# msyriac/orphics

Measured on AMD Instinct MI355X. Metric: QE kappa reconstructions/sec on 8192^2 maps, higher is better.
Workload: dtype f64

## Files before the change

### include/orphics_amd.h

```cpp
#ifndef ORPHICS_AMD_H
#define ORPHICS_AMD_H

#include <stddef.h>
#include <stdint.h>

#ifdef __cplusplus
extern "C" {
#endif

#define OA_F32 0
#define OA_F64 1

typedef struct oa_plan oa_plan;

const char* oa_last_error(void);
#define OA_ABI_VERSION 409
int oa_version(void);
int oa_device_count(void);

int oa_plan_create(int ny, int nx, int dtype, oa_plan** out);
int oa_plan_destroy(oa_plan* p);
long oa_plan_kpitch(const oa_plan* p);
long oa_plan_scratch_bytes(const oa_plan* p);
int oa_plan_set_laxes(oa_plan* p, const double* host_ly, const double* host_lx);

int oa_fft_r2c(oa_plan* p, const void* real_in, void* hc_out, double scale, int width, int rband, void* stream);
int oa_fft_c2r(oa_plan* p, const void* hc_in, void* real_out, double scale, int width, void* stream);
int oa_fft_c2r_windowed(oa_plan* p, const void* hc_in, void* real_out, double scale, const void* window_real, void* stream);
int oa_fft_c2c(oa_plan* p, const void* full_in, void* full_out, int inverse, double scale, void* stream);
int oa_fft_pass(oa_plan* p, int pass_id, const void* in, void* out, int width, void* stream);

int oa_fft_cols(oa_plan* p, const void* hc_in, void* hc_out, int inverse, double scale, int width, void* stream);
int oa_qe_rows(oa_plan* p, const void* gx, const void* gy, const void* h, void* px, void* py, double scale,
               int accumulate, int win, int wout, int mrow, void* stream);

int oa_qe_legs_cols(oa_plan* p, const void* kX, const void* kY, const void* FG, const void* FH, void* gx, void* gy, void* h,
                    int width, int rband, void* stream);
int oa_qe_map_legs_cols(oa_plan* p, const void* real_map, const void* FG, const void* FH, void* gx, void* gy, void* h,
                        int width, int rband, void* stream);
int oa_qe_cols_div(oa_plan* p, const void* px_rows, const void* py_rows, const void* Fnorm, void* out, int accumulate,
                   int width, int rband, void* stream);

int oa_plan_set_filters(oa_plan* p, const void* FG, const void* FH, const void* Fnorm, int leg_cols, int kappa_cols,
                        int leg_rows, int kappa_rows, int mrow);
int oa_plan_set_col_grid(oa_plan* p, int mcol);
int oa_plan_col_grid(const oa_plan* p);
int oa_plan_band_grid(const oa_plan* p, int* my, int* mx);
int oa_qe_band_bind(oa_plan* p, int nfilters, const void* const* host_filters, int nnorms, const void* const* host_Fnorm, int leg_cols,
                    int kappa_cols, int leg_rows, int kappa_rows, int mrow, int mcol, int max_leg_planes);
int oa_qe_band_grid(const oa_plan* p, int* my, int* mx);
int oa_plan_rsplit(const oa_plan* p);
int oa_plan_div_fused(const oa_plan* p);
enum { OA_OPT_MC_BATCH = 1, OA_OPT_MV_BATCH = 2, OA_OPT_MV_ROWBATCH = 3, OA_OPT_MV_CHAIN = 4, OA_OPT_DIV_BIN = 5, OA_OPT_WIN_FUSED = 6 };
int oa_plan_set_option(oa_plan* p, int option, int value);
int oa_plan_set_bins(oa_plan* p, const int32_t* ids_hc, int nids, double norm, void* stream);
void* oa_plan_kappa(oa_plan* p);
const int64_t* oa_plan_bin_counts(oa_plan* p);
int oa_qe_tt(oa_plan* p, const void* real_map, const void* kX, const void* kY, void* out_kappa_hc, int zero_outside,
             void* stream);
int oa_qe_pol(oa_plan* p, int npieces, const double* host_signs, const void* const* host_FG, const void* const* host_FH,
              const int* host_swap, const void* kX, const void* kY, const void* Fnorm, void* out, int accumulate,
              int leg_cols, int kappa_cols, int leg_rows, int kappa_rows, int mrow, int zero_outside, void* stream);
int oa_qe_mv(oa_plan* p, int nest, const int* host_npieces, const double* host_signs, const void* const* host_FG,
             const void* const* host_FH, const int* host_swap, const void* const* host_kX, const void* const* host_kY,
             const void* const* host_Fnorm, void* out, int accumulate, int leg_cols, int kappa_cols, int leg_rows, int kappa_rows,
             int mrow, int zero_outside, void* stream);
int oa_qe_mv_maps(oa_plan* p, int nmaps, const void* const* host_maps, const void* rot_c, const void* rot_s, int nest,
                  const int* host_npieces, const double* host_signs, const void* const* host_FG, const void* const* host_FH,
                  const int* host_swap, const int* host_xsrc, const int* host_ysrc, const void* const* host_Fnorm, void* out,
                  int accumulate, int leg_cols, int kappa_cols, int leg_rows, int kappa_rows, int mrow, int zero_outside, void* stream);
int oa_filter_map(oa_plan* p, const void* real_in, const void* filt_hcreal, void* real_out, void* stream);
int oa_qe_tt_moments(oa_plan* p, const void* real_map, int64_t* n, double* S, double* C, void* stream);
int oa_qe_tt_moments2(oa_plan* p, const void* real_map0, const void* real_map1, int64_t* n, double* S, double* C, void* stream);
int oa_qe_tt_splits(oa_plan* p, int nsplits, const void* const* host_kmaps, void* const* host_out, int zero_outside, void* stream);
int oa_qe_tt_split_power(oa_plan* p, int nsplits, const void* const* host_kmaps, void* out_hcreal, double norm, int zero_outside,
                         void* stream);
int oa_split_cross_power(int dtype, int nsplits, const void* const* host_kappa, void* out_hcreal, double norm, int ny, long kpitch,
                         int active_cols, int active_rows, void* stream);
int oa_mc_run(oa_plan* p, uint64_t base_seed, long sim_lo, long sim_hi, const void* covsqrt_hc, int64_t* n, double* S,
              double* C, double* meanfield_acc, void* stream);
int oa_mc_run_windowed(oa_plan* p, uint64_t base_seed, long sim_lo, long sim_hi, const void* covsqrt_hc, const void* window_real,
                       int64_t* n, double* S, double* C, double* meanfield_acc, void* stream);
int oa_mc_mv_band_bind(oa_plan* p, const void* mv_weights, long mv_wstride, int nest, const int32_t* ids_hc, int nids, int nspec_max);
int oa_mc_run_mv(oa_plan* p, uint64_t base_seed, long sim_lo, long sim_hi, const void* const* host_covsqrt, int nest, const int* host_npieces,
                 const double* host_signs, const void* const* host_FG, const void* const* host_FH, const int* host_swap, const int* host_xsrc,
                 const int* host_ysrc, const void* const* host_Fnorm, const void* mv_weights, long mv_wstride, int nspec, const int* host_a,
                 const int* host_b, const int32_t* ids_hc, int nids, const int64_t* counts, double norm, int leg_cols, int kappa_cols,
                 int leg_rows, int kappa_rows, int mrow, int64_t* n, double* S, double* C, void* stream);
int oa_mc_run_mv_windowed(oa_plan* p, uint64_t base_seed, long sim_lo, long sim_hi, const void* const* host_covsqrt, int nest,
                          const int* host_npieces, const double* host_signs, const void* const* host_FG, const void* const* host_FH,
                          const int* host_swap, const int* host_xsrc, const int* host_ysrc, const void* const* host_Fnorm, const void* mv_weights,
                          long mv_wstride, int nspec, const int* host_a, const int* host_b, const int32_t* ids_hc, int nids, const int64_t* counts,
                          double norm, int leg_cols, int kappa_cols, int leg_rows, int kappa_rows, int mrow, const void* window_real,
                          const void* rot_c, const void* rot_s, int64_t* n, double* S, double* C, double* const* host_meanfield, void* stream);
int oa_qe_tt_stage(oa_plan* p, int stage, const void* real_map, void* stream);

int oa_malloc(void** out, size_t bytes);
int oa_free(void* dptr);
int oa_memcpy(void* dst, const void* src, size_t bytes, int kind, void* stream);
int oa_memset(void* dptr, int value, size_t bytes, void* stream);
int oa_stream_synchronize(void* stream);

int oa_comm_unique_id(void* id128);
int oa_comm_init(int nranks, int rank, const void* id128, void** comm_out);
int oa_comm_destroy(void* comm);
int oa_allreduce(void* comm, void* device_buf, long count, int dtype_code, void* stream);

int oa_hc_to_full(oa_plan* p, const void* hc_in, void* full_out, void* stream);
int oa_full_to_hc(oa_plan* p, const void* full_in, void* hc_out, void* stream);
int oa_hcreal_to_full(oa_plan* p, const void* hcreal_in, void* fullreal_out, void* stream);
int oa_fullreal_to_hc(oa_plan* p, const void* fullreal_in, void* hcreal_out, void* stream);

int oa_f2power(int dtype, const void* k1, const void* k2, void* out_real, double norm, long n, void* stream);
int oa_cmul_real(int dtype, const void* k_in, const void* filt_real, void* k_out, long n, void* stream);
int oa_cmul(int dtype, const void* k_in, const void* filt_complex, void* k_out, long n, void* stream);
int oa_mul_real(int dtype, const void* a, const void* b, void* out, long n, void* stream);
int oa_axpby_real(int dtype, const void* a, const void* b, void* out, double alpha, double beta, long n, void* stream);
int oa_rot2(int dtype, const void* c, const void* s, const void* i1, const void* i2, void* o1, void* o2, long n, void* stream);

int oa_qe_legs(oa_plan* p, const void* kX, const void* kY, const void* FG, const void* FH,
               void* Gx, void* Gy, void* H, int phase_g, int phase_h, int h_times_i, void* stream);
int oa_qe_div(oa_plan* p, const void* Px, const void* Py, const void* Fnorm, void* out, int accumulate, void* stream);

int oa_lens_split(int dtype, const void* alpha, double step, int32_t* shift, void* delta, long n, void* stream);
int oa_lens_gather(oa_plan* p, const void* src, const int32_t* shift_x, const int32_t* shift_y, const void* dx, const void* dy,
                   int pow_x, int pow_y, double coef, void* out, int accumulate, void* stream);
int oa_hc_derivs(oa_plan* p, const void* hc_in, int order, void* hc_out_planes, long plane_stride, void* stream);
int oa_lens_taylor(oa_plan* p, const void* src, const void* deriv_planes, long plane_stride, int order, const int32_t* shift_x,
                   const int32_t* shift_y, const void* dx, const void* dy, void* out, void* stream);
int oa_lens_maps(oa_plan* p, int nmaps, const void* real_in, long in_stride, int order, const int32_t* shift_x, const int32_t* shift_y,
                 const void* dx, const void* dy, void* real_out, long out_stride, void* stream);
int oa_lens_maps_hc(oa_plan* p, int nmaps, const void* hc_in, long hc_stride, double scale, int order, const int32_t* shift_x,
                    const int32_t* shift_y, const void* dx, const void* dy, void* real_out, long out_stride, void* stream);
int oa_plan_release_pools(oa_plan* p);

int oa_digitize(const double* x, long n, const double* edges, int nedges, int32_t* ids, void* stream);
// ... 38 lines not shown
```

### orphics_amd/_lib.py

```python
import ctypes
import os

_HERE = os.path.dirname(os.path.abspath(__file__))
LIB_PATH = os.environ.get("ORPHICS_AMD_LIB", os.path.join(_HERE, "liborphics_amd.so"))

OA_F32 = 0
OA_F64 = 1
ABI_VERSION = 409

c_void_p = ctypes.c_void_p
c_int = ctypes.c_int
c_long = ctypes.c_long
c_double = ctypes.c_double
c_u64 = ctypes.c_uint64

SIGNATURES = {
    "oa_last_error": (ctypes.c_char_p, []),
    "oa_version": (c_int, []),
    "oa_device_count": (c_int, []),
    "oa_plan_create": (c_int, [c_int, c_int, c_int, ctypes.POINTER(c_void_p)]),
    "oa_plan_destroy": (c_int, [c_void_p]),
    "oa_plan_kpitch": (c_long, [c_void_p]),
    "oa_plan_scratch_bytes": (c_long, [c_void_p]),
    "oa_plan_set_laxes": (c_int, [c_void_p, c_void_p, c_void_p]),
    "oa_fft_r2c": (c_int, [c_void_p, c_void_p, c_void_p, c_double, c_int, c_int, c_void_p]),
    "oa_fft_c2r": (c_int, [c_void_p, c_void_p, c_void_p, c_double, c_int, c_void_p]),
    "oa_fft_c2r_windowed": (c_int, [c_void_p, c_void_p, c_void_p, c_double, c_void_p, c_void_p]),
    "oa_fft_c2c": (c_int, [c_void_p, c_void_p, c_void_p, c_int, c_double, c_void_p]),
    "oa_fft_pass": (c_int, [c_void_p, c_int, c_void_p, c_void_p, c_int, c_void_p]),
    "oa_fft_cols": (c_int, [c_void_p, c_void_p, c_void_p, c_int, c_double, c_int, c_void_p]),
    "oa_qe_rows": (c_int, [c_void_p] * 6 + [c_double, c_int, c_int, c_int, c_int, c_void_p]),
    "oa_qe_legs_cols": (c_int, [c_void_p] * 8 + [c_int, c_int, c_void_p]),
    "oa_qe_map_legs_cols": (c_int, [c_void_p] * 7 + [c_int, c_int, c_void_p]),
    "oa_qe_cols_div": (c_int, [c_void_p] * 5 + [c_int, c_int, c_int, c_void_p]),
    "oa_plan_set_filters": (c_int, [c_void_p] * 4 + [c_int] * 5),
    "oa_plan_set_col_grid": (c_int, [c_void_p, c_int]),
    "oa_plan_col_grid": (c_int, [c_void_p]),
    "oa_plan_band_grid": (c_int, [c_void_p, ctypes.POINTER(c_int), ctypes.POINTER(c_int)]),
    "oa_qe_band_bind": (c_int, [c_void_p, c_int, c_void_p, c_int, c_void_p] + [c_int] * 7),
    "oa_qe_band_grid": (c_int, [c_void_p, ctypes.POINTER(c_int), ctypes.POINTER(c_int)]),
    "oa_plan_rsplit": (c_int, [c_void_p]),
    "oa_plan_div_fused": (c_int, [c_void_p]),
    "oa_plan_set_option": (c_int, [c_void_p, c_int, c_int]),
    "oa_plan_set_bins": (c_int, [c_void_p, c_void_p, c_int, c_double, c_void_p]),
    "oa_plan_kappa": (c_void_p, [c_void_p]),
    "oa_plan_bin_counts": (c_void_p, [c_void_p]),
    "oa_qe_tt": (c_int, [c_void_p] * 5 + [c_int, c_void_p]),
    "oa_qe_pol": (c_int, [c_void_p, c_int, c_void_p, c_void_p, c_void_p, c_void_p, c_void_p, c_void_p, c_void_p, c_void_p, c_int,
                          c_int, c_int, c_int, c_int, c_int, c_int, c_void_p]),
    "oa_qe_mv": (c_int, [c_void_p, c_int] + [c_void_p] * 9 + [c_int] * 7 + [c_void_p]),
    "oa_qe_mv_maps": (c_int, [c_void_p, c_int, c_void_p, c_void_p, c_void_p, c_int] + [c_void_p] * 8 + [c_void_p] + [c_int] * 7 + [c_void_p]),
    "oa_filter_map": (c_int, [c_void_p] * 5),
    "oa_qe_tt_moments": (c_int, [c_void_p] * 6),
    "oa_qe_tt_moments2": (c_int, [c_void_p] * 7),
    "oa_qe_tt_splits": (c_int, [c_void_p, c_int, c_void_p, c_void_p, c_int, c_void_p]),
    "oa_qe_tt_split_power": (c_int, [c_void_p, c_int, c_void_p, c_void_p, c_double, c_int, c_void_p]),
    "oa_split_cross_power": (c_int, [c_int, c_int, c_void_p, c_void_p, c_double, c_int, c_long, c_int, c_int, c_void_p]),
    "oa_qe_tt_stage": (c_int, [c_void_p, c_int, c_void_p, c_void_p]),
    "oa_mc_run": (c_int, [c_void_p, c_u64, c_long, c_long, c_void_p, c_void_p, c_void_p, c_void_p, c_void_p, c_void_p]),
    "oa_mc_run_windowed": (c_int, [c_void_p, c_u64, c_long, c_long, c_void_p, c_void_p, c_void_p, c_void_p, c_void_p, c_void_p, c_void_p]),
    "oa_mc_run_mv": (c_int, [c_void_p, c_u64, c_long, c_long, c_void_p, c_int] + [c_void_p] * 9 + [c_long, c_int, c_void_p, c_void_p, c_void_p, c_int,
                             c_void_p, c_double] + [c_int] * 5 + [c_void_p] * 4),
    "oa_mc_run_mv_windowed": (c_int, [c_void_p, c_u64, c_long, c_long, c_void_p, c_int] + [c_void_p] * 9 + [c_long, c_int, c_void_p, c_void_p, c_void_p,
                                      c_int, c_void_p, c_double] + [c_int] * 5 + [c_void_p] * 8),
    "oa_mc_mv_band_bind": (c_int, [c_void_p, c_void_p, c_long, c_int, c_void_p, c_int, c_int]),
    "oa_malloc": (c_int, [ctypes.POINTER(c_void_p), ctypes.c_size_t]),
    "oa_free": (c_int, [c_void_p]),
    "oa_memcpy": (c_int, [c_void_p, c_void_p, ctypes.c_size_t, c_int, c_void_p]),
    "oa_memset": (c_int, [c_void_p, c_int, ctypes.c_size_t, c_void_p]),
    "oa_stream_synchronize": (c_int, [c_void_p]),
    "oa_comm_unique_id": (c_int, [c_void_p]),
    "oa_comm_init": (c_int, [c_int, c_int, c_void_p, ctypes.POINTER(c_void_p)]),
    "oa_comm_destroy": (c_int, [c_void_p]),
    "oa_allreduce": (c_int, [c_void_p, c_void_p, c_long, c_int, c_void_p]),
    "oa_hc_to_full": (c_int, [c_void_p, c_void_p, c_void_p, c_void_p]),
    "oa_full_to_hc": (c_int, [c_void_p, c_void_p, c_void_p, c_void_p]),
    "oa_hcreal_to_full": (c_int, [c_void_p, c_void_p, c_void_p, c_void_p]),
    "oa_fullreal_to_hc": (c_int, [c_void_p, c_void_p, c_void_p, c_void_p]),
    "oa_f2power": (c_int, [c_int, c_void_p, c_void_p, c_void_p, c_double, c_long, c_void_p]),
    "oa_cmul_real": (c_int, [c_int, c_void_p, c_void_p, c_void_p, c_long, c_void_p]),
    "oa_cmul": (c_int, [c_int, c_void_p, c_void_p, c_void_p, c_long, c_void_p]),
    "oa_mul_real": (c_int, [c_int, c_void_p, c_void_p, c_void_p, c_long, c_void_p]),
    "oa_axpby_real": (c_int, [c_int, c_void_p, c_void_p, c_void_p, c_double, c_double, c_long, c_void_p]),
    "oa_rot2": (c_int, [c_int, c_void_p, c_void_p, c_void_p, c_void_p, c_void_p, c_void_p, c_long, c_void_p]),
    "oa_qe_legs": (c_int, [c_void_p] * 8 + [c_int, c_int, c_int, c_void_p]),
    "oa_qe_div": (c_int, [c_void_p, c_void_p, c_void_p, c_void_p, c_void_p, c_int, c_void_p]),
    "oa_lens_split": (c_int, [c_int, c_void_p, c_double, c_void_p, c_void_p, c_long, c_void_p]),
    "oa_lens_maps": (c_int, [c_void_p, c_int, c_void_p, c_long, c_int, c_void_p, c_void_p, c_void_p, c_void_p, c_void_p, c_long, c_void_p]),
    "oa_lens_maps_hc": (c_int, [c_void_p, c_int, c_void_p, c_long, c_double, c_int, c_void_p, c_void_p, c_void_p, c_void_p, c_void_p, c_long, c_void_p]),
    "oa_plan_release_pools": (c_int, [c_void_p]),
    "oa_lens_gather": (c_int, [c_void_p] * 6 + [c_int, c_int, c_double, c_void_p, c_int, c_void_p]),
# ... 67 lines not shown
```

### orphics_amd/csrc/common.hpp

```cpp
#pragma once
#include <hip/hip_runtime.h>
#include <cstdio>
#include <cstring>
#include <string>
#include "../../include/orphics_amd.h"
#include "cx.hpp"

namespace oa {

std::string& last_error_ref();

inline int fail(const std::string& msg) {
    last_error_ref() = msg;
    return 1;
}

#define OA_HIP(expr)                                                                              \
    do {                                                                                          \
        hipError_t _e = (expr);                                                                   \
        if (_e != hipSuccess)                                                                     \
            return ::oa::fail(std::string(#expr) + ": " + hipGetErrorString(_e) + " (" + __FILE__ + \
                              ":" + std::to_string(__LINE__) + ")");                              \
    } while (0)

#define OA_REQUIRE(cond, msg)                         \
    do {                                              \
        if (!(cond)) return ::oa::fail(std::string(msg)); \
    } while (0)

#define OA_LAUNCH_CHECK() OA_HIP(hipGetLastError())

template <typename T, int N>
struct alignas(sizeof(T) * N > 16 ? 16 : sizeof(T) * N) Arr {
    T v[N];
};

struct DivBinFuse {
    const int32_t* ids; long ipitch;
    const int32_t* ids_t;
    const void* fn_t;
    int tab_logc, tab_rows;
    double pnorm; int nids, nxh;
    double* part;
    long part_cap;
    double* sums;
    unsigned* ticket;
    const int64_t* mcounts; int64_t* n; double* S; double* C;
    int store;
    int gx;
    bool done;
};

inline int flat_grid(long units, int block = 256, int cap = 8192) {
    long g = (units + block - 1) / block;
    if (g < 1) g = 1;
    if (g > cap) g = cap;
    return (int)g;
}

}

struct oa_plan {
    int ny, nx, logNy, logNx, dtype, device;
    long kp;
    void* tw_x;
    void* tw_y;
    void* scratch;
    size_t scratch_bytes;
    void* ly;
    void* lx;
    void* lyd;
    void* lxd;
    double* ly64;
    double* lx64;
    bool have_laxes;
    bool pow2;
    oa_plan* inner;
    int My, Mx;
    void* chirp_y; void* chirp_x;
    void* cz_bhat; void* cz_a; void* cz_f;
    void* cz_full;
    bool mixed;
    void* mr_twx; void* mr_twxh; void* mr_twy;
    void* pipe;
    void* rq8c[5];
    void* tw_y_small[16];
    void* tw_y_m3[16];
};

namespace oa {
int plan_ensure_scratch(oa_plan* p, size_t bytes);
int czt_setup(oa_plan* p);
void czt_release(oa_plan* p);
int czt_c2c(oa_plan* p, const void* in, void* out, int inverse, double scale, hipStream_t st);
int czt_r2c(oa_plan* p, const void* real_in, void* hc_out, double scale, hipStream_t st);
int czt_c2r(oa_plan* p, const void* hc_in, void* real_out, double scale, hipStream_t st);
bool mixed_sides_ok(int ny, int nx);
int mixed_setup(oa_plan* p);
void mixed_release(oa_plan* p);
int mixed_c2c(oa_plan* p, const void* in, void* out, int inverse, double scale, hipStream_t st);
int mixed_r2c(oa_plan* p, const void* real_in, void* hc_out, double scale, hipStream_t st);
int mixed_c2r(oa_plan* p, const void* hc_in, void* real_out, double scale, hipStream_t st);
int mixed_c2r_windowed(oa_plan* p, const void* hc_in, void* real_out, double scale, const void* window, hipStream_t st);
int mixed_cols_inverse(oa_plan* p, const void* hc_in, void* hc_out, hipStream_t st);
int mixed_lens_derivs(oa_plan* p, int nmaps, const void* real_in, long in_stride, void* k0, void* hc_pool, void* real_pool, int nd, hipStream_t st,
                      const void* hc_in, long hc_stride, double hc_scale);
void pipeline_release(oa_plan* p);
long work_pitch(const oa_plan* p, int w);
int bin_power_moments(int dtype, const void* k, double norm, const int32_t* ids, long n, int nids, long hp, int nxh, double* sums,
                      int64_t* counts, void* scratch, int active_cols, int active_rows, unsigned* ticket,
                      const int64_t* mcounts, int64_t* mn, double* S, double* C, hipStream_t st, int nbatch = 1, long kstride = 0);
int stack_add_region(int dtype, const void* x, double* acc, int ny, long kp, int w, int rb, hipStream_t st, int nbatch = 1, long xstride = 0);
int band_rot2(int dtype, const void* c, const void* s, void* q, void* u, int ny, long kp, int w, int rb, hipStream_t st);
int stack_add_region_multi(int dtype, const void* k, long kstride, const void* wt, long wstride, int nest, double* const* acc, double* acc_mv,
                           int ny, long kp, int w, int rb, hipStream_t st);
int grf_mix_teb_to_tqu(oa_plan* p, uint64_t seed, uint64_t sid0, const void* const* cs, const void* rot_c, const void* rot_s, void* const* out,
                       hipStream_t st);
int plan_ensure_col_grid(oa_plan* p, int my);
int qe_rsplit_lr(const oa_plan* p, int my, int width, int wout, int mrow);
int qe_map_legs_cols_w(oa_plan* p, const void* map, const void* FG, const void* FH, void* gx, void* gy, void* h, int width,
                       int rband, long pl, hipStream_t st, int stages = 7, int my = 0, int lr = 0, const void* fgh = nullptr);
long qe_fband_table_entries(const oa_plan* p, int width, int my);
int qe_fband_pack_w(oa_plan* p, const void* FG, const void* FH, void* out, int width, int rband, int my, hipStream_t st);
int qe_legs_cols_w(oa_plan* p, const void* kX, const void* kY, const void* FG, const void* FH, void* gx, void* gy, void* h,
                   int width, int rband, long pl, hipStream_t st, int my = 0);
int pack_tiles(const oa_plan* p, const void* src, void* dst, int rows, int logc, int width, int elem_bytes, hipStream_t st);
int div_tile_logc(const oa_plan* p, int rows);
int qe_lens_derivs_w(oa_plan* p, int nmaps, const void* real_in, long in_stride, void* k0, void* hc_pool, void* real_pool, int nd, hipStream_t st,
                     const void* hc_in = nullptr, long hc_stride = 0, double hc_scale = 1.0);
int qe_windowed_rows_w(oa_plan* p, const void* hc_in, void* cols_tmp, const void* window, int width, long pl, double scale, hipStream_t st,
                       void* out = nullptr, int nz = 0, long in_moff = 0, long out_moff = 0);
int qe_fwd_cols_batch_w(oa_plan* p, const void* in, long pin, void* out, int B, long in_moff, long out_moff, int width, int rband, hipStream_t st);
int qe_legs_subset_w(oa_plan* p, const void* src, const void* F, void* a, void* b, int subset, int width, int rband, long pl,
                     hipStream_t st, int my = 0);
int qe_cols_div_batch_w(oa_plan* p, const void* pa, const void* pb, const void* Fn, void* out, void* tmp, int nmaps, long in_moff,
                        long fn_moff, long out_moff, int width, int rband, long pk, hipStream_t st, int my = 0, DivBinFuse* fuse = nullptr);
int sum_region(int dtype, const void* parts, long part_stride, int nparts, void* out, int accumulate, int ny, long kp, int w, int rb,
               hipStream_t st);
int qe_legs_batch_w(oa_plan* p, const void* src0, long off1, long off2, unsigned long long srcsel, const void* const* ftab,
                    int ngrad, int nh, void* pool, long ostride, int width, int rband, long pl, hipStream_t st, int my = 0, int selbits = 2,
                    int* finished = nullptr);
int qe_rows_batch_w(oa_plan* p, const void* gx, const void* gy, const void* h, void* px, void* py, double scale, int win, int wout, int mrow,
                    long pl, long pk, hipStream_t st, int my, int nmaps, long in_moff, long h_moff, long out_moff);
int qe_rows_table_w(oa_plan* p, int n, const void* const* gx, const void* const* gy, const void* const* h, void* const* px, void* const* py,
                    const double* scales, void* dev_tab, int upload, int accumulate, int win, int wout, int mrow, long pl, long pk, hipStream_t st,
                    int my);
size_t qe_rows_table_entry_bytes(const oa_plan* p);
int qe_rows_chain_w(oa_plan* p, int nest, int total, const void* const* gx, const void* const* gy, const void* const* h, void* const* px,
                    void* const* py, const double* scales, const int* first, const int* count, void* dev_tab, int upload, int win, int wout, int mrow,
                    long pl, long pk, hipStream_t st, int my);
int grf_hc_band_batch(oa_plan* p, uint64_t seed, uint64_t stream_id, int nreal, const void* covsqrt_hc, void* hc_out, long zstride,
                      int width, int rband, hipStream_t stream);
int moments_add_binned_multi(const double* sums, const int64_t* counts, int nspec, int nids, int64_t* n, double* S, double* C, hipStream_t st);
int bin_power_multi_check(const char* who, int dtype, int nfields, bool have_w, int nspec, const int* host_a, const int* host_b, int nids);
int qe_legs_pass2_w(oa_plan* p, void* pool, int nplanes, long stride, int width, long pl, hipStream_t st, int my = 0);
int qe_rows_w(oa_plan* p, const void* gx, const void* gy, const void* h, void* px, void* py, double scale, int accumulate,
              int win, int wout, int mrow, long pl, long pk, hipStream_t st, int my = 0, int lr = 0);
int qe_cols_div_w(oa_plan* p, const void* pa, const void* pb, const void* Fn, void* out, int accumulate, int width, int rband,
                  long pk, hipStream_t st, int my = 0, DivBinFuse* fuse = nullptr);
int qe_tt_pair_w(oa_plan* p, const void* map0, const void* map1, const void* FG, const void* FH, const void* Fn, void* c0, void* c1,
                 void* c2, void* g0, void* g1, void* out0, void* out1, int wl, int wk, int rl, int rk, int mrow, int my, long pl, long pk,
                 hipStream_t st, DivBinFuse* fuse = nullptr, const void* fgh = nullptr);
int band_map_r2c(oa_plan* p, const void* map, void* rowbuf, int wl, int rl, void* dst, int dny, long dkp, hipStream_t st);
size_t band_map_scratch_bytes(const oa_plan* p, int wl, int rl);
int band_maps_r2c(oa_plan* p, int nmaps, const void* const* maps, const void* rot_c, const void* rot_s, void* scratch, int wl, int rl, void* dst,
                  long dstride, int dny, long dkp, hipStream_t st);
size_t band_maps_scratch_bytes(const oa_plan* p, int nmaps, int wl, int rl);
int band_win_r2c(oa_plan* p, int B, const void* hc_in, long in_bstride, const void* window, double scale, void* scratch, int single, int wl, int rl,
                 void* dst, long dstride, int dny, long dkp, hipStream_t st);
bool band_rows_win_ok(const oa_plan* p);
int band_copy(int kind, const void* src, long spitch, int sny, void* dst, long dpitch, int dny, int w, int r, double scale, hipStream_t st);
int band_zero_outside(int dtype, void* out, int ny, long kp, int w, int r, hipStream_t st);
int band_stack_add(int dtype, const void* src, long spitch, int sny, int nbatch, long sstride, double* acc, long apitch, int any, int w, int r,
                   hipStream_t st);
int band_embed(int dtype, const void* const* dev_srcs, int n, long spitch, int sny, void* dst, long dstride, long dpitch, int dny, int w, int r,
               hipStream_t st);
int band_scatter(int dtype, const void* src, long spitch, int sny, void* out, long okp, int ony, int w, int r, int mode, hipStream_t st);
int band_scatter_batch(int dtype, const void* src, long sstride, int nplanes, long spitch, int sny, void* const* dev_outs, long okp, int ony, int w,
                       int r, int zero, hipStream_t st);
int band_split_power(int dtype, int nsplits, const void* src, long sstride, long spitch, int sny, void* out_real, long okp, int ony, int w, int r,
                     double norm, int zero, hipStream_t st);
int grf_band_inner(oa_plan* p, uint64_t seed, uint64_t stream_id, int nreal, const void* covsqrt_hc, void* out, int my, long okp, long zstride,
                   int width, int rband, hipStream_t stream);
}
#define OA_NEED_POW2(p, what) \
    OA_REQUIRE((p)->pow2, what ": needs power-of-two map sides (other sizes: oa_fft_r2c / oa_fft_c2r / oa_fft_c2c and the modular oa_qe_legs / oa_mul_real / oa_qe_div calls)")
```

### orphics_amd/csrc/fft.hip

```cpp
#include <cmath>
#include <vector>
#include "fft_launch.hpp"
#include "fft_r2c_w64.hpp"
#include "fft_r2c_rs4096.hpp"
#include "fft_divbin.hpp"

namespace oa {

template <typename T, int MODE, class SEQ>
__global__ __launch_bounds__(row_maxnt<SEQ>(), waves_per_eu<T>()) void row_fft_kernel(RowArgs<T> a) {
    GpuCtx c{oa_dyn_smem};
    row_fft_body<T, MODE, SEQ>(c, a);
}

#ifndef OA_W64_OCC
#define OA_W64_OCC 1
#endif
__global__ __launch_bounds__(64, OA_W64_OCC) void row_r2c_w64_kernel(RowW64Args a) {
    GpuCtx c{oa_dyn_smem};
    row_r2c_w64_body(c, a);
}

template <typename T, class SEQ, int LR, bool PF>
__global__ __launch_bounds__(row_maxnt<SEQ>(), (sizeof(T) == 8 || PF ? 2 : 3)) void row_r2c_rsplit_kernel(RowArgs<T> a) {
// ... 363 lines not shown
                    dispatch_nz<S>(qe_first_stage_nz(a.logL, S::rget(0), a.win), [&](auto nzc) {
                        go(row_qe_kernel<T, S, decltype(nzc)::value>, dim3(grid), nt, smem, a);
                    });
                } else {
                    go(row_qe_kernel<T, S, 0>, dim3(grid), nt, smem, a);
                }
            } else {
                if (!rc) rc = fail("fft: unsupported row length");
            }
        });
        if (!ok && !rc) rc = fail("fft: unsupported row length");
    }
    template <typename T>
    void row_qe_pair8(int pairs, int M, const RowQeArgs<T>& a) {
        const bool ok = dispatch_rq8(M, a.win, a.lr, a.chain != nullptr, [&](auto ac, auto nzc, auto lay, auto ch) {
            constexpr int A = decltype(ac)::value;
            if (ch.value && !a.tab) { if (!rc) rc = fail("fft: estimator chains need a table"); return; }
            if (!a.rq8c) { if (!rc) rc = fail("fft: the 8-point row stage needs the constants of its grid"); return; }
            go(row_qe8_kernel<T, A, decltype(nzc)::value, decltype(lay)::value, decltype(ch)::value>, dim3(pairs), 64 * A, rq8_lds_bytes<T, A, decltype(ch)::value>(), a);
        });
        if (!ok && !rc) rc = fail("fft: unsupported row grid / layout for the 8-point row stage");
    }
    template <typename T>
    void row_qe_pair(int grid, int nt, size_t smem, const RowQeArgs<T>& a) {
        const bool ok = dispatch_seq(a.logL, [&](auto seq) {
            using S = decltype(seq);
            if constexpr (seq_logl<S>() >= 10 && seq_logl<S>() <= 13) {
                if (nt != pair_nt<S>()) { if (!rc) rc = fail("fft: pair row stage launched with the wrong workgroup size"); return; }
                dispatch_pair_nz<S>(pair_first_stage_nz(a.logL, S::rget(0), a.win), [&](auto nzc) {
                    if (a.chain) {
                        if constexpr (seq_logl<S>() <= 12) { if (a.lr == 0 && a.tab) go(row_qe_chain_kernel<T, S, decltype(nzc)::value>, dim3(grid), nt, smem, a); else if (!rc) rc = fail("fft: estimator chains need natural-order planes and a table"); }
                        else if (!rc) rc = fail("fft: estimator chains: unsupported row grid");
                    } else
                    if (a.lr == 2) go(row_qe_pair_kernel<T, S, decltype(nzc)::value, 2>, dim3(grid), nt, smem, a);
                    else if (a.lr == 3) {
                        if constexpr (seq_logl<S>() == 11 && sizeof(T) == 8) go(row_qe_pair_kernel<T, S, decltype(nzc)::value, 3>, dim3(grid), nt, smem, a);
                        else if (!rc) rc = fail("fft: the R = 8 layout of the pair row stage is built for float64 on 2048-point row grids");
                    } else if (a.lr == 0) go(row_qe_pair_kernel<T, S, decltype(nzc)::value, 0>, dim3(grid), nt, smem, a);
                    else if (!rc) rc = fail("fft: unsupported R-layout of the pair row stage");
                });
            } else if (!rc) rc = fail("fft: unsupported row grid for the pair row stage");
        });
        if (!ok && !rc) rc = fail("fft: unsupported row grid");
    }
    template <typename T>
    void col_legs(int gx, int gy, int nt, size_t smem, int logL, const ColLegsArgs<T>& a) {
        if (rc) return;
        rc = launch_col_legs<T>(st, gx, gy, nt, smem, logL, a);
    }
    template <typename T>
    void col_legs_sp(int gx, int nt, size_t smem, int logL, const ColLegsArgs<T>& a) {
        if (rc) return;
        rc = launch_col_legs_sp<T>(st, gx, nt, smem, logL, a);
    }
    template <typename T>
    void col_fwdlegs(int gx, int gy, int nt, size_t smem, int logL, const ColFwdLegsArgs<T>& a) {
        if (rc) return;
        rc = launch_col_fwdlegs<T>(st, gx, gy, nt, smem, logL, a);
    }
    template <typename T>
    void col_fwdlegs_cg(int gx, int gy, int nt, size_t smem, int logL, const ColFwdLegsCgArgs<T>& a, int gz = 1) {
        if (rc) return;
        rc = launch_col_fwdlegs_cg<T>(st, gx, gy, nt, smem, logL, a, gz);
    }
    template <typename T>
    void col_div(int gx, int gy, int nt, size_t smem, int logL, const ColDivArgs<T>& a, int gz = 1) {
        const bool ok = dispatch_seq(logL, [&](auto seq) {
            using S = decltype(seq);
            if constexpr (seq_logl<S>() <= 8) {
                if (nt > col_maxnt<S>()) { if (!rc) rc = fail("fft: column workgroup size exceeds its launch bound"); return; }
                go(col_div_kernel<T, S>, dim3(gx, gy, gz), nt, smem, a);
            } else if (!rc) rc = fail("fft: unsupported column sub-length");
        });
        if (!ok && !rc) rc = fail("fft: unsupported column length");
    }
    DivBinFuse* fuse = nullptr;
    template <class K, typename T>
    void go_fused(K kern, int gx, int gz, int nt, size_t smem, ColDivArgs<T> a) {
        {
            const hipError_t e = ensure_dyn_lds(reinterpret_cast<const void*>(kern), smem);
            if (e != hipSuccess) { rc = fail(std::string("hipFuncSetAttribute: ") + hipGetErrorString(e)); return; }
        }
        fuse->gx = gx;
        if (!fuse->store) a.out = nullptr;
        const bool tabs = fuse->tab_logc == a.logC && fuse->tab_rows == a.ny;
        a.Fn_t = (tabs && a.fn_moff == 0) ? (const T*)fuse->fn_t : nullptr;
        if (!tabs) fuse->ids_t = nullptr;
        hipLaunchKernelGGL(kern, dim3(gx, 1, gz), dim3(nt), smem, st, a, *fuse);
        hipError_t e = hipGetLastError();
        if (e != hipSuccess) rc = fail(std::string("fft launch: ") + hipGetErrorString(e));
        fuse->done = true;
    }
    template <typename T>
    bool col_div_sp(int gx, size_t smem, int logL, const ColDivArgs<T>& a, int gz = 1) {
        if (rc) return true;
        const int lt = Fft2dPlan<T>::div_lt(), nt = (1 << lt) / EPT;
        const bool narrow = lt < (sizeof(T) == 4 ? 14 : 13);
        constexpr int lc11 = sizeof(T) == 4 ? 3 : 2, lc10 = lc11 + 1;
        if (fuse && !a.accumulate && (long)gx * gz * fuse->nids <= fuse->part_cap && (logL == 10 || logL == 11 || (logL == 12 && !narrow)) &&
            (size_t)(nt / 64) * fuse->nids * sizeof(double) <= ((size_t)1 << lt) * sizeof(cx<T>)) {
            if (logL == 12) go_fused(col_div_sp_bin_kernel<T, Seq<16, 16, 16>, lc11 - 1>, gx, gz, nt, smem, a);
            else if (logL == 11 && !narrow) go_fused(col_div_sp_bin_kernel<T, Seq<16, 16, 8>, lc11>, gx, gz, nt, smem, a);
            else if (logL == 10 && !narrow) go_fused(col_div_sp_bin_kernel<T, Seq<16, 16, 4>, lc10>, gx, gz, nt, smem, a);
            else if (logL == 11) go_fused(col_div_sp_bin_kernel<T, Seq<16, 16, 8>, lc11 - 1>, gx, gz, nt, smem, a);
            else go_fused(col_div_sp_bin_kernel<T, Seq<16, 16, 4>, lc10 - 1>, gx, gz, nt, smem, a);
            return true;
        }
        if (logL == 12 && !narrow) { go(col_div_sp_kernel<T, Seq<16, 16, 16>, lc11 - 1>, dim3(gx, 1, gz), nt, smem, a); return true; }
        if (logL == 11 && !narrow) { go(col_div_sp_kernel<T, Seq<16, 16, 8>, lc11>, dim3(gx, 1, gz), nt, smem, a); return true; }
        if (logL == 10 && !narrow) { go(col_div_sp_kernel<T, Seq<16, 16, 4>, lc10>, dim3(gx, 1, gz), nt, smem, a); return true; }
        if (logL == 11) { go(col_div_sp_kernel<T, Seq<16, 16, 8>, lc11 - 1>, dim3(gx, 1, gz), nt, smem, a); return true; }
        if (logL == 10) { go(col_div_sp_kernel<T, Seq<16, 16, 4>, lc10 - 1>, dim3(gx, 1, gz), nt, smem, a); return true; }
        return false;
    }
    template <typename T>
    void col_div3(int gx, size_t smem, int rows, const ColDivArgs<T>& a, int gz = 1) {
        if (rc) return;
        constexpr int lc = sizeof(T) == 4 ? 3 : 2;
        if (rows != 1536 && rows != 768) { rc = fail("fft: unsupported 3 x 2^k divergence grid"); return; }
        const int nt = a.NT;
        if (fuse && !a.accumulate && (long)gx * gz * fuse->nids <= fuse->part_cap &&
            (size_t)(nt / 64) * fuse->nids * sizeof(double) <= ((size_t)rows << a.logC) * sizeof(cx<T>)) {
            if (rows == 1536) go_fused(col_div3_sp_bin_kernel<T, 8, lc>, gx, gz, nt, smem, a);
            else go_fused(col_div3_sp_bin_kernel<T, 7, lc + 1>, gx, gz, nt, smem, a);
            return;
        }
        if (rows == 1536) go(col_div3_sp_kernel<T, 8, lc>, dim3(gx, 1, gz), nt, smem, a);
        else go(col_div3_sp_kernel<T, 7, lc + 1>, dim3(gx, 1, gz), nt, smem, a);
    }
    template <typename T>
    void col_deriv(int gx, int gy, int nt, size_t smem, const ColDerivArgs<T>& a, int nz) {
        const bool ok = dispatch_seq(a.logL, [&](auto seq) {
            using S = decltype(seq);
            if constexpr (seq_logl<S>() <= 8) {
                if (nt > col_maxnt<S>()) { if (!rc) rc = fail("fft: column workgroup size exceeds its launch bound"); return; }
                go(col_deriv_kernel<T, S>, dim3(gx, gy, nz), nt, smem, a);
            } else if (!rc) rc = fail("fft: unsupported column sub-length");
        });
        if (!ok && !rc) rc = fail("fft: unsupported column length");
    }
    template <typename T>
    void col(int gx, int gy, int nt, size_t smem, const ColArgs<T>& a, int nz = 1) {
        const bool ok = dispatch_seq(a.logL, [&](auto seq) {
            using S = decltype(seq);
            if constexpr (seq_logl<S>() <= 8) {
                if (nt > col_maxnt<S>()) { if (!rc) rc = fail("fft: column workgroup size exceeds its launch bound"); return; }
                go(col_fft_kernel<T, S>, dim3(gx, gy, nz), nt, smem, a);
            } else {
                if (!rc) rc = fail("fft: unsupported column sub-length");
            }
        });
        if (!ok && !rc) rc = fail("fft: unsupported column length");
    }
};

template <typename T>
static Fft2dPlan<T> view(const oa_plan* p) {
    Fft2dPlan<T> f;
    f.ny = p->ny; f.nx = p->nx; f.logNy = p->logNy; f.logNx = p->logNx; f.kp = p->kp;
    f.tw_x = (const cx<T>*)p->tw_x; f.tw_y = (const cx<T>*)p->tw_y; for (int i = 0; i < RQ8_NGRIDS; ++i) f.rq8c[i] = (const cx<T>*)p->rq8c[i];
    return f;
}
template <typename T>
static Fft2dPlan<T> coarse_view(const oa_plan* p, int my) {
    Fft2dPlan<T> f = view<T>(p);
    if (my > 0 && my < p->ny && is_pow2(my) && p->tw_y_small[ilog2(my)]) {
        f.ny = my; f.logNy = ilog2(my); f.tw_y = (const cx<T>*)p->tw_y_small[ilog2(my)]; f.ny_full = p->ny;
    } else if (my > 0 && my < p->ny && is_m3(my) && p->tw_y_m3[ilog2(my / 3)]) {
        f.ny = my; f.logNy = -1; f.tw_y = (const cx<T>*)p->tw_y_m3[ilog2(my / 3)]; f.ny_full = p->ny;
    }
    return f;
}
static bool m3_ready(const oa_plan* p, int my) { return my > 0 && my < p->ny && is_m3(my) && p->tw_y_m3[ilog2(my / 3)] && p->tw_y_small[ilog2(m3_pow2(my))]; }
int plan_ensure_col_grid(oa_plan* p, int my) {
    if (my <= 0 || my >= p->ny) return 0;
    if (is_m3(my) && my >= 96) {
        if (int rc = plan_ensure_col_grid(p, m3_pow2(my))) return rc;
    } else
    if (!is_pow2(my) || my < 32) return fail("column grid must be a power of two >= 32");
    void*& slot = is_m3(my) ? p->tw_y_m3[ilog2(my / 3)] : p->tw_y_small[ilog2(my)];
    if (slot) return 0;
    if (p->dtype == OA_F32) {
        auto t = make_twiddles<float>(my);
        OA_HIP(hipMalloc(&slot, t.size() * sizeof(cx<float>)));
        OA_HIP(hipMemcpy(slot, t.data(), t.size() * sizeof(cx<float>), hipMemcpyHostToDevice));
    } else {
        auto t = make_twiddles<double>(my);
        OA_HIP(hipMalloc(&slot, t.size() * sizeof(cx<double>)));
        OA_HIP(hipMemcpy(slot, t.data(), t.size() * sizeof(cx<double>), hipMemcpyHostToDevice));
    }
    return 0;
}

template <typename T>
static int r2c_impl(oa_plan* p, const void* in, void* out, double scale, int width, int rband, hipStream_t st) {
    if (int rc = plan_ensure_scratch(p, (size_t)p->ny * p->kp * sizeof(cx<T>))) return rc;
    HipLauncher q{st};
    view<T>(p).r2c(q, (const T*)in, (cx<T>*)out, (cx<T>*)p->scratch, (T)scale, width, rband);
    return q.rc;
}
template <typename T>
static int c2r_impl(oa_plan* p, const void* in, void* out, double scale, int width, hipStream_t st, const void* mul = nullptr) {
    if (int rc = plan_ensure_scratch(p, (size_t)p->ny * p->kp * sizeof(cx<T>))) return rc;
    HipLauncher q{st};
// ... 88 lines not shown
    const size_t plane = (size_t)p->ny * p->kp * sizeof(cx<T>);
    if (int rc = plan_ensure_scratch(p, 2 * plane)) return rc;
    HipLauncher q{st};
    auto f = view<T>(p);
    cx<T>* tA = (cx<T>*)p->scratch;
    cx<T>* tB = tA + (size_t)p->ny * p->kp;
    const int w = f.clampw(width);
    const long pw = pwork > 0 ? pwork : p->kp;
    if (lr > 0) {
        const auto cv = coarse_view<T>(p, my);
        if (is_m3(my)) {
            const int myf = m3_pow2(my);
            const long kplane3 = (long)myf * pw;
            if (stages & 1) f.rows_rsplit(q, map, tA, pw, kplane3, w, myf);
            if (stages & 4) f.legs_fband3(q, cv, (const cx<T>*)p->tw_y_small[ilog2(myf)], tA, kplane3, pw, (const T*)FG, (const T*)FH, (const T*)p->lxd,
                                          (const T*)p->lyd, (cx<T>*)gx, (cx<T>*)gy, (cx<T>*)h, width, rband, pout > 0 ? pout : p->kp, 1, 0, 0, (const cx<T>*)fgh);
            return q.rc;
        }
        const long kplane = (long)my * pw;
        if (stages & 1) f.rows_rsplit(q, map, tA, pw, kplane, w, my);
        if (stages & 4) f.legs_fband(q, cv, tA, kplane, pw, (const T*)FG, (const T*)FH, (const T*)p->lxd, (const T*)p->lyd, (cx<T>*)gx, (cx<T>*)gy,
                                     (cx<T>*)h, width, rband, pout > 0 ? pout : p->kp, 1, 0, 0, (const cx<T>*)fgh);
        return q.rc;
    }
    if (stages & 1) f.rows(q, ROW_R2C, map, p->nx / 2, tA, pw, (T)1, w);
    if (my > 0 && my < p->ny) {
        if (stages & 2) f.cols(q, tA, pw, tB, pw, w, false, (T)1, 1);
        if (stages & 4) {
            static const bool nofuse = exp_env("OA_NO_FWDLEGS_CG") != nullptr;
            const auto cv = coarse_view<T>(p, my);
            if (nofuse || !f.legs_cols_from_pass1_cg(q, cv, tB, (const T*)FG, (const T*)FH, (const T*)p->lxd, (const T*)p->lyd,
                                                     (cx<T>*)gx, (cx<T>*)gy, (cx<T>*)h, width, pw, pout)) {
                f.cols(q, tA, pw, tB, pw, w, false, (T)1, 2, 1, nullptr, nullptr, rband);
                cv.legs_cols(q, tB, tB, (const T*)FG, (const T*)FH, (const T*)p->lxd, (const T*)p->lyd, (cx<T>*)gx, (cx<T>*)gy,
                             (cx<T>*)h, width, rband, pw, pout, true);
            }
        }
    } else if (Fft2dPlan<T>::has_fwdlegs(p->logNy)) {
        if (stages & 2) f.cols(q, tA, pw, tB, pw, w, false, (T)1, 1);
        if (stages & 4)
            f.legs_cols_from_pass1(q, tB, (const T*)FG, (const T*)FH, (const T*)p->lxd, (const T*)p->lyd, (cx<T>*)gx,
                                   (cx<T>*)gy, (cx<T>*)h, width, rband, pw, pout);
    } else {
        if (stages & 2) f.cols(q, tA, pw, tB, pw, w, false, (T)1, 0, 1, nullptr, nullptr, rband);
        if (stages & 4)
            f.legs_cols(q, tB, tB, (const T*)FG, (const T*)FH, (const T*)p->lxd, (const T*)p->lyd, (cx<T>*)gx, (cx<T>*)gy,
                        (cx<T>*)h, width, rband, pw, pout);
    }
    return q.rc;
}

template <typename T>
static int cols_div_impl(oa_plan* p, const void* pa, const void* pb, const void* Fn, void* out, int accumulate,
                         int width, int rband, hipStream_t st, long pin = 0, int my = 0, DivBinFuse* fuse = nullptr) {
    const size_t plane = (size_t)p->ny * p->kp * sizeof(cx<T>);
    if (int rc = plan_ensure_scratch(p, 2 * plane)) return rc;
    HipLauncher q{st};
    q.fuse = fuse;
    cx<T>* tA = (cx<T>*)p->scratch;
    cx<T>* tB = tA + (size_t)p->ny * p->kp;
    if (is_m3(my)) {
        if (!m3_ready(p, my)) return fail("fft: 3 x 2^k column grid without its tables");
        coarse_view<T>(p, my).cols_div3(q, (const cx<T>*)pa, (const cx<T>*)pb, (const T*)Fn, (const T*)p->lxd, (const T*)p->lyd, (cx<T>*)out, accumulate,
                                        width, rband, pin);
        return q.rc;
    }
    coarse_view<T>(p, my).cols_div(q, (const cx<T>*)pa, (const cx<T>*)pb, (const T*)Fn, (const T*)p->lxd, (const T*)p->lyd,
                                   (cx<T>*)out, tA, tB, accumulate, width, rband, pin);
    return q.rc;
}

template <typename T>
static int cols_div_batch_impl(oa_plan* p, const void* pa, const void* pb, const void* Fn, void* out, void* tmp, int nmaps, long in_moff,
                               long fn_moff, long out_moff, int width, int rband, hipStream_t st, long pin, int my, DivBinFuse* fuse = nullptr) {
    HipLauncher q{st};
    q.fuse = fuse;
    cx<T>* tA = (cx<T>*)tmp;
    cx<T>* tB = tA + (in_moff >> 1);
    coarse_view<T>(p, my).cols_div(q, (const cx<T>*)pa, (const cx<T>*)pb, (const T*)Fn, (const T*)p->lxd, (const T*)p->lyd, (cx<T>*)out, tA,
                                   tB, 0, width, rband, pin, nmaps, in_moff, in_moff, out_moff, fn_moff);
    return q.rc;
}

template <typename T>
static int qe_tt_pair_impl(oa_plan* p, const void* map0, const void* map1, const void* FG, const void* FH, const void* Fn, void* c0,
                           void* c1, void* c2, void* g0, void* g1, void* out0, void* out1, int wl, int wk, int rl, int rk, int mrow,
                           int my, long pl, long pk, hipStream_t st, DivBinFuse* fuse, const void* fgh) {
    auto f = view<T>(p);
    const int lr = rsplit_lr<T>(p, my, wl, wk, mrow);
    const bool m3 = is_m3(my);
    if (m3 && !(lr && m3_ready(p, my))) return -1;
    if (!m3)
    if (!(my > 0 && my < p->ny && is_pow2(my) && p->tw_y_small[ilog2(my)]) || !(lr || Fft2dPlan<T>::has_fwdlegs_cg(p->logNy, my))) return -1;
    const auto cv = coarse_view<T>(p, my);
    const int wi = f.clampw(wl), wo = f.clampw(wk);
    if (mrow < 0) { mrow = Fft2dPlan<T>::row_grid_min(p->nx, wi, wo); if (2L * wi + wo > mrow) mrow = 0; }
    if (!cv.rows_qe_is_pair(wi, wo, mrow)) return -1;
    const long ms = (long)p->ny * pl, cms = (long)my * pl, gms = (long)my * pk;
    if (2 * ms > (long)p->ny * p->kp || 2 * gms > (long)p->ny * p->kp) return -1;
    const size_t plane = (size_t)p->ny * p->kp * sizeof(cx<T>);
    if (int rc = plan_ensure_scratch(p, 2 * plane)) return rc;
    HipLauncher q{st};
    q.fuse = fuse;
    cx<T>* tA = (cx<T>*)p->scratch;
    cx<T>* tB = tA + (size_t)p->ny * p->kp;
    const double s = 1.0 / ((double)p->ny * p->nx), sy = (double)p->ny / my;
    if (lr) {
        const int myf = m3 ? m3_pow2(my) : my;
        const long kplane = (long)myf * pl;
        f.rows_rsplit(q, map0, tA, pl, kplane, wi, myf);
        f.rows_rsplit(q, map1, tA + ms, pl, kplane, wi, myf);
        if (m3) f.legs_fband3(q, cv, (const cx<T>*)p->tw_y_small[ilog2(myf)], tA, kplane, pl, (const T*)FG, (const T*)FH, (const T*)p->lxd, (const T*)p->lyd,
                              (cx<T>*)c0, (cx<T>*)c1, (cx<T>*)c2, wl, rl, pl, 2, ms, cms, (const cx<T>*)fgh);
        else
        f.legs_fband(q, cv, tA, kplane, pl, (const T*)FG, (const T*)FH, (const T*)p->lxd, (const T*)p->lyd, (cx<T>*)c0, (cx<T>*)c1, (cx<T>*)c2, wl, rl,
                     pl, 2, ms, cms, (const cx<T>*)fgh);
        cv.rows_qe(q, (const cx<T>*)c0, (const cx<T>*)c1, (const cx<T>*)c2, (cx<T>*)g0, (cx<T>*)g1, (T)(s * s * sy), 0, wi, wo, mrow, pl, pk, 2, cms, gms,
                   -1, nullptr, lr);
        if (m3) cv.cols_div3(q, (const cx<T>*)g0, (const cx<T>*)g1, (const T*)Fn, (const T*)p->lxd, (const T*)p->lyd, (cx<T>*)out0, 0, wk, rk, pk, 2, gms,
                             (long)((cx<T>*)out1 - (cx<T>*)out0));
        else
        cv.cols_div(q, (const cx<T>*)g0, (const cx<T>*)g1, (const T*)Fn, (const T*)p->lxd, (const T*)p->lyd, (cx<T>*)out0, tA, tB, 0, wk, rk, pk, 2,
                    gms, gms, (long)((cx<T>*)out1 - (cx<T>*)out0));
        return q.rc;
    }
    f.rows(q, ROW_R2C, map0, p->nx / 2, tA, pl, (T)1, wi);
    f.rows(q, ROW_R2C, map1, p->nx / 2, tA + ms, pl, (T)1, wi);
    const cx<T>* ins[2] = {tA, tA + ms};
    cx<T>* outs[2] = {tB, tB + ms};
    f.cols(q, tA, pl, tB, pl, wi, false, (T)1, 1, 2, ins, outs);
    if (!f.legs_cols_from_pass1_cg(q, cv, tB, (const T*)FG, (const T*)FH, (const T*)p->lxd, (const T*)p->lyd, (cx<T>*)c0, (cx<T>*)c1,
                                   (cx<T>*)c2, wl, pl, pl, 2, ms, cms))
        return -1;
    cv.rows_qe(q, (const cx<T>*)c0, (const cx<T>*)c1, (const cx<T>*)c2, (cx<T>*)g0, (cx<T>*)g1, (T)(s * s * sy), 0, wi, wo, mrow, pl, pk, 2, cms, gms);
    cv.cols_div(q, (const cx<T>*)g0, (const cx<T>*)g1, (const T*)Fn, (const T*)p->lxd, (const T*)p->lyd, (cx<T>*)out0, tA, tB, 0, wk, rk, pk, 2,
                gms, gms, (long)((cx<T>*)out1 - (cx<T>*)out0));
    return q.rc;
}
int qe_tt_pair_w(oa_plan* p, const void* map0, const void* map1, const void* FG, const void* FH, const void* Fn, void* c0, void* c1,
                 void* c2, void* g0, void* g1, void* out0, void* out1, int wl, int wk, int rl, int rk, int mrow, int my, long pl, long pk,
                 hipStream_t st, DivBinFuse* fuse, const void* fgh) {
    return p->dtype == OA_F32 ? qe_tt_pair_impl<float>(p, map0, map1, FG, FH, Fn, c0, c1, c2, g0, g1, out0, out1, wl, wk, rl, rk, mrow, my, pl, pk, st, fuse, fgh)
                              : qe_tt_pair_impl<double>(p, map0, map1, FG, FH, Fn, c0, c1, c2, g0, g1, out0, out1, wl, wk, rl, rk, mrow, my, pl, pk, st, fuse, fgh);
}
template <typename T>
static int fband_pack_impl(oa_plan* p, const void* FG, const void* FH, void* out, int width, int rband, int my, hipStream_t st) {
    HipLauncher q{st};
    auto f = view<T>(p);
    const auto cv = coarse_view<T>(p, my);
    if (is_m3(my)) {
        if (!m3_ready(p, my)) return fail("fft: 3 x 2^k column grid without its tables");
        f.legs_fband3(q, cv, (const cx<T>*)p->tw_y_small[ilog2(m3_pow2(my))], nullptr, 0, 0, (const T*)FG, (const T*)FH, (const T*)p->lxd, (const T*)p->lyd,
                      nullptr, nullptr, nullptr, width, rband, 0, 1, 0, 0, nullptr, (cx<T>*)out);
        return q.rc;
    }
    f.legs_fband(q, cv, nullptr, 0, 0, (const T*)FG, (const T*)FH, (const T*)p->lxd, (const T*)p->lyd, nullptr, nullptr, nullptr, width, rband, 0, 1, 0, 0,
                 nullptr, (cx<T>*)out);
    return q.rc;
}
long qe_fband_table_entries(const oa_plan* p, int width, int my) {
    if (is_m3(my))
        return p->dtype == OA_F32 ? view<float>(p).fband3_table_entries(coarse_view<float>(p, my), width)
                                  : view<double>(p).fband3_table_entries(coarse_view<double>(p, my), width);
    return p->dtype == OA_F32 ? view<float>(p).fband_table_entries(coarse_view<float>(p, my), width)
                              : view<double>(p).fband_table_entries(coarse_view<double>(p, my), width);
}
int qe_fband_pack_w(oa_plan* p, const void* FG, const void* FH, void* out, int width, int rband, int my, hipStream_t st) {
    return p->dtype == OA_F32 ? fband_pack_impl<float>(p, FG, FH, out, width, rband, my, st) : fband_pack_impl<double>(p, FG, FH, out, width, rband, my, st);
}

long work_pitch(const oa_plan* p, int w) {
    return p->dtype == OA_F32 ? view<float>(p).work_pitch(w) : view<double>(p).work_pitch(w);
}
int qe_map_legs_cols_w(oa_plan* p, const void* map, const void* FG, const void* FH, void* gx, void* gy, void* h, int width,
                       int rband, long pl, hipStream_t st, int stages, int my, int lr, const void* fgh) {
    return p->dtype == OA_F32 ? map_legs_cols_impl<float>(p, map, FG, FH, gx, gy, h, width, rband, st, pl, pl, stages, my, lr, fgh)
                              : map_legs_cols_impl<double>(p, map, FG, FH, gx, gy, h, width, rband, st, pl, pl, stages, my, lr, fgh);
}
template <typename T>
static int windowed_rows_impl(oa_plan* p, const void* hc_in, void* cols_tmp, const void* window, int width, long pl, double scale, hipStream_t st,
                              void* out, int nz, long in_moff, long out_moff) {
    const size_t plane = (size_t)p->ny * p->kp * sizeof(cx<T>);
    if (int rc = plan_ensure_scratch(p, 2 * plane)) return rc;
    HipLauncher q{st};
    auto f = view<T>(p);
    if (nz > 0) f.cols(q, (const cx<T>*)hc_in, p->kp, (cx<T>*)cols_tmp, p->kp, p->nx / 2 + 1, true, (T)1, 0, 1, nullptr, nullptr, 0, false, -1, nz, in_moff, in_moff);
    else f.cols(q, (const cx<T>*)hc_in, p->kp, (cx<T>*)cols_tmp, p->kp, p->nx / 2 + 1, true, (T)1);
    f.rows(q, ROW_WIN, cols_tmp, p->kp, out ? out : p->scratch, pl > 0 ? pl : p->kp, (T)scale, f.clampw(width), window, nz, in_moff, out_moff);
    return q.rc;
}
int qe_windowed_rows_w(oa_plan* p, const void* hc_in, void* cols_tmp, const void* window, int width, long pl, double scale, hipStream_t st, void* out,
                       int nz, long in_moff, long out_moff) {
    return p->dtype == OA_F32 ? windowed_rows_impl<float>(p, hc_in, cols_tmp, window, width, pl, scale, st, out, nz, in_moff, out_moff)
                              : windowed_rows_impl<double>(p, hc_in, cols_tmp, window, width, pl, scale, st, out, nz, in_moff, out_moff);
}
template <typename T>
static int fwd_cols_batch_impl(oa_plan* p, const void* in, long pin, void* out, int B, long in_moff, long out_moff, int width, int rband, hipStream_t st) {
    HipLauncher q{st};
    auto f = view<T>(p);
    f.cols(q, (const cx<T>*)in, pin, (cx<T>*)out, p->kp, f.clampw(width), false, (T)1, 0, 1, nullptr, nullptr, rband, false, -1, B, in_moff, out_moff);
    return q.rc;
}
int qe_fwd_cols_batch_w(oa_plan* p, const void* in, long pin, void* out, int B, long in_moff, long out_moff, int width, int rband, hipStream_t st) {
    return p->dtype == OA_F32 ? fwd_cols_batch_impl<float>(p, in, pin, out, B, in_moff, out_moff, width, rband, st)
                              : fwd_cols_batch_impl<double>(p, in, pin, out, B, in_moff, out_moff, width, rband, st);
}
template <typename T>
static int lens_derivs_impl(oa_plan* p, int nmaps, const void* real_in, long in_stride, void* k0, void* hc_pool, void* real_pool, int nd,
                            hipStream_t st, const void* hc_in, long hc_stride, double hc_scale) {
    const size_t plane = (size_t)p->ny * p->kp * sizeof(cx<T>);
    if (int rc = plan_ensure_scratch(p, plane)) return rc;
    HipLauncher q{st};
    auto f = view<T>(p);
    const long hcp = (long)p->ny * p->kp, rp = (long)p->ny * (p->nx / 2);
    const cx<T>* src = hc_in ? (const cx<T>*)hc_in : (const cx<T>*)k0;
    const long sstride = hc_in ? hc_stride : hcp;
    const int d00 = hc_in ? 1 : 0;
    if (!hc_in)
        for (int m = 0; m < nmaps; ++m)
            f.r2c(q, (const T*)real_in + (long)m * in_stride, (cx<T>*)k0 + (long)m * hcp, (cx<T>*)p->scratch, (T)1);
    const int order = (int)((std::sqrt(8.0 * (nd + 1) + 1.0) - 1.0) / 2.0 + 0.5);
    const double cscale = hc_in ? hc_scale : 1.0 / ((double)p->ny * p->nx);
    for (int m = 0; m < nmaps; ++m)
        for (int b = 0; b < order; ++b) {
            const int a0 = (b == 0 && !d00) ? 1 : 0, na = order - b - a0;
            if (na <= 0) continue;
// ... 250 lines not shown
```

### orphics_amd/csrc/fft_divbin.hpp

```cpp
#pragma once
#include "fft_launch.hpp"

namespace oa {

#if defined(__HIP_DEVICE_COMPILE__) && !(defined(__gfx942__) || defined(__gfx950__))
#error "DivBinTail: the ticket hand-over relies on gfx942 / gfx950 behaviour (agent-scope relaxed atomic stores are sc1 write-through, stores count in vmcnt)"
#endif

template <int CTRL>
__device__ __forceinline__ double dpp_f64(double v) {
    const unsigned long long u = __builtin_bit_cast(unsigned long long, v);
    const int lo = __builtin_amdgcn_update_dpp(0, (int)(unsigned)u, CTRL, 0xf, 0xf, false);
    const int hi = __builtin_amdgcn_update_dpp(0, (int)(unsigned)(u >> 32), CTRL, 0xf, 0xf, false);
    return __builtin_bit_cast(double, ((unsigned long long)(unsigned)hi << 32) | (unsigned long long)(unsigned)lo);
}
__device__ __forceinline__ double readlane_f64(double v, int lane) {
    const unsigned long long u = __builtin_bit_cast(unsigned long long, v);
    const unsigned lo = (unsigned)__builtin_amdgcn_readlane((int)(unsigned)u, lane);
    const unsigned hi = (unsigned)__builtin_amdgcn_readlane((int)(unsigned)(u >> 32), lane);
    return __builtin_bit_cast(double, ((unsigned long long)hi << 32) | (unsigned long long)lo);
}
__device__ __forceinline__ double wave_total_f64(double v) {
    v += dpp_f64<0xB1>(v);
    v += dpp_f64<0x4E>(v);
    v += dpp_f64<0x141>(v);
    v += dpp_f64<0x140>(v);
    return ((readlane_f64(v, 0) + readlane_f64(v, 16)) + readlane_f64(v, 32)) + readlane_f64(v, 48);
}

template <typename T>
struct DivBinTail {
    static constexpr bool active = true;
    DivBinFuse f;
    double* rows = nullptr;

    __device__ __forceinline__ void begin(GpuCtx&, void* lds) {
        rows = reinterpret_cast<double*>(lds);
        const int nw = blockDim.x >> 6;
        for (int i = threadIdx.x; i < nw * f.nids; i += blockDim.x) rows[i] = 0.0;
    }
    __device__ __forceinline__ int id_at(unsigned yfull, int col) const { return f.ids[(long)yfull * f.ipitch + col]; }
    __device__ __forceinline__ bool packed_ids() const { return f.ids_t != nullptr; }
    __device__ __forceinline__ int id_at_t(long i) const { return f.ids_t[i]; }
    __device__ __forceinline__ void add(GpuCtx&, int id, T pw, int col) {
        const int m = (col == 0 || col == f.nxh) ? 1 : (col < f.nxh ? 2 : 0);
        const bool ok = id >= 0 && id < f.nids && m > 0;
        const double v = ok ? (double)(pw * (T)f.pnorm) * (double)m : 0.0;
        const int lane = threadIdx.x & 63;
        double* row = rows + (threadIdx.x >> 6) * f.nids;
        unsigned long long act = __ballot(ok);
        while (act) {
            const int leader = __ffsll((long long)act) - 1;
            const int lid = __shfl(id, leader, 64);
            const bool mine = ok && id == lid;
            const unsigned long long mm = __ballot(mine);
            const double sv = wave_total_f64(mine ? v : 0.0);
            if (lane == leader) row[lid] += sv;
            act &= ~mm;
        }
    }
    __device__ __forceinline__ void finish(GpuCtx&) {
        __shared__ int s_last;
        const int t = threadIdx.x, nt = blockDim.x, nw = nt >> 6, nids = f.nids;
        __syncthreads();
        const long wg = (long)blockIdx.z * gridDim.x + blockIdx.x;
        for (int i = t; i < nids; i += nt) {
            double s = 0.0;
            for (int k = 0; k < nw; ++k) s += rows[k * nids + i];
            __hip_atomic_store(f.part + wg * nids + i, s, __ATOMIC_RELAXED, __HIP_MEMORY_SCOPE_AGENT);
        }
        asm volatile("s_waitcnt vmcnt(0)" ::: "memory");
        __syncthreads();
        if (t == 0)
            s_last = (__hip_atomic_fetch_add(f.ticket, 1u, OA_TICKET_ORDER, __HIP_MEMORY_SCOPE_AGENT) == gridDim.x * gridDim.z - 1) ? 1 : 0;
        __syncthreads();
        if (!s_last) return;
        const int d = nids - 2;
        int NI = 1;
        while (NI < nids && NI < nt) NI <<= 1;
        const int G = nt / NI > 0 ? nt / NI : 1, gi = t / NI, ii = t - gi * NI;
        double* red = rows;
        const int gx = (int)gridDim.x;
        for (int z = 0; z < (int)gridDim.z; ++z) {
            for (int i0 = 0; i0 < nids; i0 += NI) {
                const int i = i0 + ii;
                __syncthreads();
                if (gi < G) {
                    double s = 0.0;
                    if (i < nids) {
                        const double* pz = f.part + ((long)z * gx) * nids + i;
                        int b = gi;
                        for (; b + 3 * G < gx; b += 4 * G) {
                            const double p0 = __hip_atomic_load(pz + (long)b * nids, __ATOMIC_RELAXED, __HIP_MEMORY_SCOPE_AGENT);
                            const double p1 = __hip_atomic_load(pz + (long)(b + G) * nids, __ATOMIC_RELAXED, __HIP_MEMORY_SCOPE_AGENT);
                            const double p2 = __hip_atomic_load(pz + (long)(b + 2 * G) * nids, __ATOMIC_RELAXED, __HIP_MEMORY_SCOPE_AGENT);
                            const double p3 = __hip_atomic_load(pz + (long)(b + 3 * G) * nids, __ATOMIC_RELAXED, __HIP_MEMORY_SCOPE_AGENT);
                            s += (p0 + p1) + (p2 + p3);
                        }
                        for (; b < gx; b += G) s += __hip_atomic_load(pz + (long)b * nids, __ATOMIC_RELAXED, __HIP_MEMORY_SCOPE_AGENT);
                    }
                    red[gi * NI + ii] = s;
                }
                __syncthreads();
                double tot = 0.0;
                if (gi == 0 && i < nids) {
                    for (int k = 0; k < G; ++k) tot += red[k * NI + ii];
                    f.sums[(long)z * nids + i] = tot;
                }
                __syncthreads();
                if (gi == 0 && i >= 1 && i <= d) red[G * NI + i - 1] = tot / (double)f.mcounts[i];
            }
            __syncthreads();
            const double* bv = red + G * NI;
            if (f.S) {
                for (int a = t; a < d; a += nt) f.S[a] += bv[a];
                for (long e = t; e < (long)d * d; e += nt) {
                    const int ra = (int)(e / d), cb = (int)(e - (long)ra * d);
                    f.C[e] += bv[ra] * bv[cb];
                }
            }
        }
        if (t == 0) {
            if (f.n) f.n[0] += (int64_t)gridDim.z;
            __hip_atomic_store(f.ticket, 0u, __ATOMIC_RELAXED, __HIP_MEMORY_SCOPE_AGENT);
        }
    }
};

}
```

### orphics_amd/csrc/fft_kernels.hpp

```cpp
#pragma once
#include <type_traits>
#include "cx.hpp"

namespace oa {

constexpr int EPT = 16;
#ifndef OA_COL_LOGC
#define OA_COL_LOGC 5
#endif
constexpr int COL_LOGC = OA_COL_LOGC;

enum RowMode { ROW_R2C = 0, ROW_C2R = 1, ROW_C2C_F = 2, ROW_C2C_I = 3, ROW_WIN = 4 };

template <typename T>
OA_HD cx<T> w16(int k) {
    const T c1 = (T)0.92387953251128673848L;
    const T s1 = (T)0.38268343236508978178L;
    const T h = (T)0.70710678118654752440L;
    switch (k) {
        case 0: return mk<T>((T)1, (T)0);
        case 1: return mk<T>(c1, -s1);
        case 2: return mk<T>(h, -h);
        case 3: return mk<T>(s1, -c1);
        case 4: return mk<T>((T)0, (T)-1);
// ... 1399 lines not shown
    constexpr int LQ = 16;
    static_assert(Ns == LQ && NB == 4, "col_fwdlegs_cg: needs 16 positions per butterfly and 4 butterflies per thread");
    constexpr int logC = COL_LOGC;
    constexpr int NT = (1 << (logL + COL_LOGC)) / EPT;
    static_assert(NT == 4 << COL_LOGC, "col_fwdlegs_cg: a thread owns positions q + 4 u of one column");
    const int tid = ctx.tid();
    const int c0 = ctx.bid_x() << logC;
    const long g = ctx.bid_y();
    int ncols = a.width - c0;
    if (ncols > (1 << logC)) ncols = 1 << logC;
    cx<T> gv[EPT];
    cx<T>* twl = s + (1 << (logL + logC));
    cx<T>* ex = twl + tw_lds_size(logL);
    tw_lds_fill<T>(ctx, twl, a.tw, a.logTw, logL, NT);
    ctx.sync();
    const long imo = ctx.bid_z() ? a.in_moff : 0, omo = ctx.bid_z() ? a.out_moff : 0;
    const ColLoad<T> ld{a.in + imo + g * a.pitch + c0, (unsigned)(a.n1f * a.pitch), ncols, false};
    col_pipeline_to_regs<T, SEQF>(ctx, s, gv, tid, NT, logC, twl, logL, ld);
    const int c = tid & ((1 << logC) - 1), q = tid >> logC;
    const bool ok = c < ncols;
    const T lx = ok ? a.lxd[c0 + c] : (T)0;
    for (int leg = 0; leg < 3; ++leg) {
        cx<T> v[4];
#pragma unroll
        for (int u = 0; u < 4; ++u) {
            const int j = q + 4 * u;
            const bool low = j < LQ / 2;
            const cx<T> x = low ? gv[u * RL] : gv[u * RL + RL - 1];
            const int k2 = low ? j : (L - LQ) + j;
            const unsigned y = (unsigned)g + (unsigned)k2 * (unsigned)a.n1f;
            cx<T> val = mk<T>((T)0, (T)0);
            if (ok) {
                const unsigned fi = y * (unsigned)a.fpitch + (unsigned)(c0 + c);
                if (leg == 0) val = x * a.FH[fi];
                else if (leg == 1) val = mul_pi(x * a.FG[fi]) * lx;
                else val = mul_pi(x * a.FG[fi]) * a.lyd[y];
            }
            v[u] = swp(val);
        }
        Dft<T, 4>::run(v);
#pragma unroll
        for (int aa = 1; aa < 4; ++aa) {
            const int e = q * aa;
            const cx<T> w = w16<T>(e & 7);
            v[aa] = v[aa] * (e >= 8 ? mk<T>(-w.x, -w.y) : w);
        }
        if (leg) ctx.sync();
#pragma unroll
        for (int aa = 0; aa < 4; ++aa) ex[((q * 4 + aa) << logC) + c] = v[aa];
        ctx.sync();
        cx<T>* out = (leg == 0 ? a.h : (leg == 1 ? a.gx : a.gy)) + omo + (g * LQ) * a.opitch + c0;
#pragma unroll
        for (int aa = 0; aa < 4; ++aa) {
            cx<T> t[4];
#pragma unroll
            for (int qq = 0; qq < 4; ++qq) t[qq] = ex[((qq * 4 + aa) << logC) + c];
            Dft<T, 4>::run(t);
            const int y = aa + 4 * q;
            cx<T> r = (q == 0 ? t[0] : (q == 1 ? t[1] : (q == 2 ? t[2] : t[3])));
            r = swp(r * a.twc[(unsigned)g * (unsigned)y]);
            if (ok) out[(unsigned)y * (unsigned)a.opitch + (unsigned)c] = r;
        }
    }
}

template <typename T>
struct ColDivArgs {
    const cx<T>* A; const cx<T>* B;
    const T* Fn;
    const T* lxd; const T* lyd;
    cx<T>* out;
    long pitch;
    long opitch;
    int width, logC, NT;
    const cx<T>* tw;
    int logTw;
    long in_gs, in_ns, out_gs, out_ks;
    int accumulate;
    int rband, ny;
    int yshift;
    long in_moff, out_moff;
    long fn_moff;
    const T* Fn_t;
};

struct NoDivTail {
    static constexpr bool active = false;
    template <class Ctx> OA_HD void begin(Ctx&, void*) {}
    OA_HD int id_at(unsigned, int) const { return -1; }
    OA_HD bool packed_ids() const { return false; }
    OA_HD int id_at_t(long) const { return -1; }
    template <class Ctx, typename T> OA_HD void add(Ctx&, int, T, int) {}
    template <class Ctx> OA_HD void finish(Ctx&) {}
};

template <typename T, class SEQ, class Ctx, int LOGC = COL_LOGC, class Tail = NoDivTail>
OA_HD void col_div_body(Ctx& ctx, const ColDivArgs<T>& a, Tail tail = Tail{}) {
    cx<T>* s = reinterpret_cast<cx<T>*>(ctx.smem());
    constexpr int logL = Log2x<SEQ::r0>::v + Log2x<SEQ::r1>::v + Log2x<SEQ::r2>::v + Log2x<SEQ::r3>::v;
    constexpr int n = SEQ::n;
    constexpr int RL = SEQ::get(n - 1), LRL = Log2x<RL>::v, NB = EPT / RL;
    constexpr int logNs = logL - LRL;
    constexpr int logC = LOGC;
    constexpr int NT = ((1 << (seq_total_log<SEQ>() + LOGC)) / EPT) > 0 ? ((1 << (seq_total_log<SEQ>() + LOGC)) / EPT) : 1;
    const int tid = ctx.tid();
    int tile = ctx.bid_x();
    if ((sizeof(cx<T>) << LOGC) < 128) {
        const int nt = ctx.grid_x(), base = tile & ~15, r = tile & 15;
        if (base + 16 <= nt) tile = base + 2 * (r & 7) + (r >> 3);
    }
    const int c0 = tile << logC;
    const long g = ctx.bid_y();
    int ncols = a.width - c0;
    if (ncols > (1 << logC)) ncols = 1 << logC;
    cx<T> va[EPT], vb[EPT];
    cx<T>* twl = s + (1 << (logL + logC));
    tw_lds_fill<T>(ctx, twl, a.tw, a.logTw, logL, NT);
    ctx.sync();
    const long zmap = ctx.bid_z();
    const long imo = zmap * a.in_moff, omo = zmap * a.out_moff;
    const ColLoad<T> la{a.A + imo + g * a.in_gs * a.pitch + c0, (unsigned)(a.in_ns * a.pitch), ncols, false};
    const ColLoad<T> lb{a.B + imo + g * a.in_gs * a.pitch + c0, (unsigned)(a.in_ns * a.pitch), ncols, false};
    if constexpr (n == 2) {
        constexpr int R0 = SEQ::get(0);
        constexpr int l0 = Log2x<R0>::v;
        stage_in<T, R0, false, true>(s, va, tid, NT, logL, logC, 0, 0, twl, logL, la);
        stage_in<T, R0, false, true>(s, vb, tid, NT, logL, logC, 0, 0, twl, logL, lb);
        stage_out<T, R0, false, false>(s, va, tid, NT, logL, logC, 0, 0, NoStore{});
        ctx.sync();
        stage_in<T, RL, false, false>(s, va, tid, NT, logL, logC, 0, l0, twl, logL, NoLoad{});
        ctx.sync();
        stage_out<T, R0, false, false>(s, vb, tid, NT, logL, logC, 0, 0, NoStore{});
        ctx.sync();
        stage_in<T, RL, false, false>(s, vb, tid, NT, logL, logC, 0, l0, twl, logL, NoLoad{});
    } else {
        col_pipeline_to_regs<T, SEQ>(ctx, s, va, tid, NT, logC, twl, logL, la);
        ctx.sync();
        col_pipeline_to_regs<T, SEQ>(ctx, s, vb, tid, NT, logC, twl, logL, lb);
    }
    const long oorg = g * a.out_gs * a.opitch + c0;
    const T* Fnb = a.Fn + zmap * a.fn_moff + oorg;
    cx<T>* outb = a.out + omo + oorg;
    const unsigned ostr = (unsigned)(a.out_ks * a.opitch);
    if constexpr (Tail::active) {
        ctx.sync();
        tail.begin(ctx, s);
        ctx.sync();
        T pw[EPT];
        int idv[EPT];
#pragma unroll
        for (int u = 0; u < NB; ++u) {
            const int b = tid + u * NT;
            const int c = b & ((1 << logC) - 1), j = b >> logC;
            const bool cok = c < ncols;
            const int kq = j & ((1 << logNs) - 1);
            const int base = ((j - kq) << LRL) + kq;
            const T lx = cok ? a.lxd[c0 + c] : (T)0;
#pragma unroll
            for (int t = 0; t < RL; ++t) {
                const int k = base + (t << logNs);
                const unsigned y = (unsigned)(g * a.out_gs) + (unsigned)k * (unsigned)a.out_ks;
                const bool ok = cok && !(a.rband && (int)y >= a.rband && (int)y <= a.ny - a.rband);
                const unsigned up = (a.yshift && y >= (unsigned)(a.ny >> 1)) ? (unsigned)a.yshift : 0u;
                const unsigned i = (unsigned)k * ostr + (unsigned)c + up * (unsigned)a.opitch;
                pw[u * RL + t] = (T)0;
                idv[u * RL + t] = -1;
                if (ok) {
                    const long ti_ = (((long)tile << logL) + k) * (1 << logC) + c;
                    const T fn = a.Fn_t ? a.Fn_t[ti_] : Fnb[i];
                    cx<T> d = mul_pi(va[u * RL + t] * lx + vb[u * RL + t] * a.lyd[y + up]) * fn;
                    if (a.out) {
                        if (a.accumulate) d = d + outb[i];
                        outb[i] = d;
                    }
                    pw[u * RL + t] = d.x * d.x + d.y * d.y;
                    idv[u * RL + t] = tail.packed_ids() ? tail.id_at_t((((long)tile << logL) + k) * (1 << logC) + c) : tail.id_at(y + up, c0 + c);
                }
            }
        }
#pragma unroll
        for (int u = 0; u < NB; ++u) {
            const int c = (tid + u * NT) & ((1 << logC) - 1);
#pragma unroll
            for (int t = 0; t < RL; ++t) tail.add(ctx, idv[u * RL + t], pw[u * RL + t], c0 + c);
        }
        tail.finish(ctx);
    } else {
#pragma unroll
    for (int u = 0; u < NB; ++u) {
        const int b = tid + u * NT;
        const int c = b & ((1 << logC) - 1), j = b >> logC;
        if (c >= ncols) continue;
        const int kq = j & ((1 << logNs) - 1);
        const int base = ((j - kq) << LRL) + kq;
        const T lx = a.lxd[c0 + c];
#pragma unroll
        for (int t = 0; t < RL; ++t) {
            const int k = base + (t << logNs);
            const unsigned y = (unsigned)(g * a.out_gs) + (unsigned)k * (unsigned)a.out_ks;
            if (a.rband && (int)y >= a.rband && (int)y <= a.ny - a.rband) continue;
            const unsigned up = (a.yshift && y >= (unsigned)(a.ny >> 1)) ? (unsigned)a.yshift : 0u;
            const unsigned i = (unsigned)k * ostr + (unsigned)c + up * (unsigned)a.opitch;
            cx<T> d = mul_pi(va[u * RL + t] * lx + vb[u * RL + t] * a.lyd[y + up]) * Fnb[i];
            if (a.accumulate) d = d + outb[i];
            outb[i] = d;
        }
    }
    }
}

template <typename T> OA_HD void dft6(cx<T>* v) {
    const T hs = (T)0.86602540378443864676L;
    cx<T> e[3] = {v[0], v[2], v[4]}, o[3] = {v[1], v[3], v[5]};
    auto d3 = [&](cx<T>* z) {
        const cx<T> s = z[1] + z[2], d = (z[1] - z[2]) * hs, m = z[0] - s * (T)0.5;
        z[0] = z[0] + s; z[1] = add_mi(m, d); z[2] = add_pi(m, d);
    };
    d3(e); d3(o);
    o[1] = o[1] * mk<T>((T)0.5, -hs);
    o[2] = o[2] * mk<T>((T)-0.5, -hs);
#pragma unroll
    for (int q = 0; q < 3; ++q) { v[q] = e[q] + o[q]; v[q + 3] = e[q] - o[q]; }
}

template <typename T, int LOGQ, int LOGC, class Ctx, class Tail = NoDivTail>
OA_HD void col_div3_body(Ctx& ctx, const ColDivArgs<T>& a, Tail tail = Tail{}) {
    cx<T>* s = reinterpret_cast<cx<T>*>(ctx.smem());
    using SEQ = typename SeqOf<LOGQ>::type;
    static_assert(SEQ::n == 2, "col_div3: two-stage sub-transforms");
    constexpr int R0 = SEQ::get(0), R1 = SEQ::get(1), l0 = Log2x<R0>::v;
    constexpr int Q = 1 << LOGQ, N = 6 * Q, C = 1 << LOGC, logC = LOGC;
    constexpr int NTS = (Q << LOGC) / EPT, NT = 6 * NTS;
    constexpr int NIT = ((Q << LOGC) + NT - 1) / NT;
    const int tid = ctx.tid();
    int tile = ctx.bid_x();
    if ((sizeof(cx<T>) << LOGC) < 128) {
        const int nt = ctx.grid_x(), base = tile & ~15, r = tile & 15;
        if (base + 16 <= nt) tile = base + 2 * (r & 7) + (r >> 3);
    }
    const int c0 = tile << logC;
    int ncols = a.width - c0;
    if (ncols > C) ncols = C;
    cx<T>* twl = s + (N << logC);
    tw_lds_fill_mul<T>(ctx, twl, a.tw, 6, LOGQ, NT);
    const long zmap = ctx.bid_z();
    const long imo = zmap * a.in_moff, omo = zmap * a.out_moff;
    const int grp = tid / NTS, tq = tid - grp * NTS;
    cx<T>* sr = s + grp * (Q << logC);
    const ColLoad<T> la{a.A + imo + (long)grp * a.pitch + c0, (unsigned)(6 * a.pitch), ncols, false};
    const ColLoad<T> lb{a.B + imo + (long)grp * a.pitch + c0, (unsigned)(6 * a.pitch), ncols, false};
    int pk[NIT], pc[NIT];
    bool pv[NIT];
    cx<T> w1[NIT], w2[NIT], w4[NIT];
#pragma unroll
    for (int it = 0; it < NIT; ++it) {
        const int i = tid + it * NT;
        pv[it] = i < (Q << logC);
        const int ii = pv[it] ? i : tid;
        pc[it] = ii & (C - 1); pk[it] = ii >> logC;
        w1[it] = ldg(a.tw + pk[it]); w2[it] = ldg(a.tw + 2 * pk[it]); w4[it] = ldg(a.tw + 4 * pk[it]);
    }
    cx<T> va[EPT], vb[EPT];
    cx<T> xa[NIT][6], xb[NIT][6];
    stage_in<T, R0, false, true>(s, va, tq, NTS, LOGQ, logC, 0, 0, twl, LOGQ, la);
    stage_in<T, R0, false, true>(s, vb, tq, NTS, LOGQ, logC, 0, 0, twl, LOGQ, lb);
    ctx.sync();
    auto finish = [&](cx<T>* v, cx<T> (*x)[6]) {
        stage_out<T, R0, false, false>(sr, v, tq, NTS, LOGQ, logC, 0, 0, NoStore{});
        ctx.sync();
        stage<T, R1, false, false, false>(ctx, sr, tq, NTS, LOGQ, logC, 0, l0, twl, LOGQ, NoLoad{}, NoStore{});
        ctx.sync();
#pragma unroll
        for (int it = 0; it < NIT; ++it) {
#pragma unroll
            for (int r = 0; r < 6; ++r) x[it][r] = s[((r * Q + pk[it]) << logC) + pc[it]];
            const cx<T> w3 = w1[it] * w2[it], w5 = w4[it] * w1[it];
            x[it][1] = x[it][1] * w1[it]; x[it][2] = x[it][2] * w2[it]; x[it][3] = x[it][3] * w3;
            x[it][4] = x[it][4] * w4[it]; x[it][5] = x[it][5] * w5;
            dft6<T>(x[it]);
        }
    };
    finish(va, xa);
    ctx.sync();
    finish(vb, xb);
    const T* Fnb = a.Fn + zmap * a.fn_moff + c0;
    cx<T>* outb = a.out + omo + c0;
    if constexpr (Tail::active) {
        ctx.sync();
        tail.begin(ctx, s);
        ctx.sync();
        T pw[NIT * 6];
        int idv[NIT * 6];
#pragma unroll
        for (int it = 0; it < NIT; ++it) {
            const int c = pc[it], k = pk[it];
            const bool cok = pv[it] && c < ncols;
            const T lx = cok ? a.lxd[c0 + c] : (T)0;
#pragma unroll
            for (int q = 0; q < 6; ++q) {
                const unsigned y = (unsigned)(k + Q * q);
                const bool ok = cok && !(a.rband && (int)y >= a.rband && (int)y <= a.ny - a.rband);
                const unsigned up = (a.yshift && y >= (unsigned)(N >> 1)) ? (unsigned)a.yshift : 0u;
                const unsigned i = (y + up) * (unsigned)a.opitch + (unsigned)c;
                pw[it * 6 + q] = (T)0;
                idv[it * 6 + q] = -1;
                if (ok) {
                    const long ti_ = ((long)tile * N + y) * C + c;
                    const T fn = a.Fn_t ? a.Fn_t[ti_] : Fnb[i];
                    cx<T> d = mul_pi(xa[it][q] * lx + xb[it][q] * a.lyd[y + up]) * fn;
                    if (a.out) {
                        if (a.accumulate) d = d + outb[i];
                        outb[i] = d;
                    }
                    pw[it * 6 + q] = d.x * d.x + d.y * d.y;
                    idv[it * 6 + q] = tail.packed_ids() ? tail.id_at_t(ti_) : tail.id_at(y + up, c0 + c);
                }
            }
        }
#pragma unroll
        for (int it = 0; it < NIT; ++it) {
#pragma unroll
            for (int q = 0; q < 6; ++q) tail.add(ctx, idv[it * 6 + q], pw[it * 6 + q], c0 + pc[it]);
        }
        tail.finish(ctx);
    } else {
#pragma unroll
        for (int it = 0; it < NIT; ++it) {
            const int c = pc[it], k = pk[it];
            if (!pv[it] || c >= ncols) continue;
            const T lx = a.lxd[c0 + c];
#pragma unroll
            for (int q = 0; q < 6; ++q) {
                const unsigned y = (unsigned)(k + Q * q);
                if (a.rband && (int)y >= a.rband && (int)y <= a.ny - a.rband) continue;
                const unsigned up = (a.yshift && y >= (unsigned)(N >> 1)) ? (unsigned)a.yshift : 0u;
                const unsigned i = (y + up) * (unsigned)a.opitch + (unsigned)c;
                cx<T> d = mul_pi(xa[it][q] * lx + xb[it][q] * a.lyd[y + up]) * Fnb[i];
                if (a.accumulate) d = d + outb[i];
                outb[i] = d;
            }
        }
    }
}

template <typename T>
struct ColDerivArgs {
    const cx<T>* in;
    cx<T>* out;
    long in_mstride, out_pstride, pitch;
    int width, nd, logL;
    int zbase;
    int bonly;
    const cx<T>* tw;
    int logTw;
    long in_ns, out_gs;
    const T* lxd; const T* lyd;
};

template <typename T, bool BONLY = false>
struct ColDerivLoad {
    static constexpr bool reads_lds = false;
    const cx<T>* base;
    unsigned nstride;
    int ncols;
    const T* fx;
    const T* fy;
    T cr, ci;
    int q;
    template <typename U> OA_HD cx<U> get(int n, int c) const {
        const int cc = c < ncols ? c : ncols - 1;
        const cx<U> v = base[(unsigned)n * nstride + (unsigned)cc];
        cx<U> x;
        if constexpr (BONLY) {
            const U f = c < ncols ? fy[n] : (U)0;
            const bool odd = (q & 1) != 0;
            const U sr = (q == 1 || q == 2) ? -f : f, si = (q >= 2) ? -f : f;
            x = mk<U>((odd ? v.y : v.x) * sr, (odd ? v.x : v.y) * si);
        } else {
            const U f = c < ncols ? fx[cc] * fy[n] : (U)0;
            x = mk<U>((v.x * cr - v.y * ci) * f, (v.x * ci + v.y * cr) * f);
        }
        return swp(x);
    }
};

template <typename T, class SEQ, class Ctx>
OA_HD void col_deriv_body(Ctx& ctx, const ColDerivArgs<T>& a) {
    cx<T>* s = reinterpret_cast<cx<T>*>(ctx.smem());
    const int tid = ctx.tid();
    constexpr int CLC = COL_LOGC;
    constexpr int logL = seq_total_log<SEQ>();
    constexpr int CNT = ((1 << (logL + COL_LOGC)) / EPT) > 0 ? ((1 << (logL + COL_LOGC)) / EPT) : 1;
    const int c0 = ctx.bid_x() << CLC;
    const long g = ctx.bid_y();
    int ncols = a.width - c0;
    if (ncols > (1 << CLC)) ncols = 1 << CLC;
    cx<T>* twl = s + (1 << (logL + CLC));
    cx<T>* ti = twl + tw_lds_size(logL);
    T* fy = reinterpret_cast<T*>(ti + (1 << logL));
    T* fx = fy + (1 << logL);
    const int z = a.zbase + ctx.bid_z(), m = z / a.nd, d = z - m * a.nd;
    int n = 1;
    while ((n + 1) * (n + 2) / 2 - 1 <= d) ++n;
    int b = d - (n * (n + 1) / 2 - 1), aa = n - b;
    if (a.bonly) { b = d; aa = 0; n = d; }
    tw_lds_fill<T>(ctx, twl, a.tw, a.logTw, logL, CNT);
    for (int i = tid; i < (1 << logL); i += CNT) {
        ti[i] = a.tw[(unsigned)g * (unsigned)i];
        const T ly = a.lyd[(unsigned)g + (unsigned)i * (unsigned)a.in_ns];
        T f = (T)1;
        for (int k = 0; k < b; ++k) f *= ly;
        fy[i] = f;
    }
    for (int i = tid; i < (1 << CLC); i += CNT) {
        const T lx = (c0 + i < a.width) ? a.lxd[c0 + i] : (T)0;
        T f = (T)1;
        for (int k = 0; k < aa; ++k) f *= lx;
        fx[i] = f;
    }
    ctx.sync();
    const int q = n & 3;
    const T cr = (T)((q == 0) - (q == 2)), ci = (T)((q == 1) - (q == 3));
    const ColStore<T> st{a.out + (long)ctx.bid_z() * a.out_pstride + g * a.out_gs * a.pitch + c0, (unsigned)a.pitch, ncols, true, ti, (unsigned)g, (T)1,
                         0, 0, 0, 0};
    if (a.bonly) {
// ... 38 lines not shown
```

### orphics_amd/csrc/fft_plan.hpp

```cpp
#pragma once
#include <cmath>
#include <cstdlib>
#include <vector>
#include "fft_kernels.hpp"
#include "fft_fband.hpp"
#include "fft_rowqe8.hpp"

namespace oa {

template <typename T>
inline std::vector<cx<T>> make_twiddles(int M) {
    std::vector<cx<T>> t((size_t)M);
    const long double tau = 6.283185307179586476925286766559005768L;
    for (int k = 0; k < M; ++k) {
        long double a = tau * (long double)k / (long double)M;
        t[(size_t)k].x = (T)cosl(a);
        t[(size_t)k].y = (T)(-sinl(a));
    }
    return t;
}

inline long kpitch_for(int nx) { return nx / 2 + 16; }

inline bool is_pow2(int v) { return v > 0 && (v & (v - 1)) == 0; }
// ... 326 lines not shown
        const int tiles = (width + C - 1) / C;
        ColFwdLegsArgs<T> a{};
        a.in = p1; a.FG = FG; a.FH = FH; a.lxd = lxd; a.lyd = lyd; a.gx = gx; a.gy = gy; a.h = h;
        a.pitch = pi; a.fpitch = kp; a.opitch = po;
        a.width = width; a.tw = tw_y; a.logTw = logNy; a.n1f = N1f; a.rband = clampr(rband); a.ny = ny;
        q.col_fwdlegs(tiles, (int)N1f, (int)((L * C) / EPT), ((size_t)L * C + tw_lds_size(logL) + L) * sizeof(cx<T>), logL, a);
        cx<T>* outs[3] = {gx, gy, h};
        const cx<T>* ins[3] = {gx, gy, h};
        cols(q, gx, po, gx, po, width, true, (T)1, 2, 3, ins, outs, 0, true);
        return true;
    }

    static bool has_fwdlegs_cg(int logNy, int my) {
        const int logL = logNy / 2;
        return logL == 6 && my > 0 && (my >> (logNy - logL)) == 16;
    }
    template <class Launcher>
    bool legs_cols_from_pass1_cg(Launcher& q, const Fft2dPlan<T>& cv, const cx<T>* p1, const T* FG, const T* FH, const T* lxd,
                                 const T* lyd, cx<T>* gx, cx<T>* gy, cx<T>* h, int wmax, long pin, long pout, int nmaps = 1,
                                 long in_moff = 0, long out_moff = 0) const {
        if (!has_fwdlegs_cg(logNy, cv.ny)) return false;
        const long pi = pin > 0 ? pin : kp, po = pout > 0 ? pout : kp;
        const int logL = logNy / 2, logN1f = logNy - logL;
        const long L = 1L << logL, N1f = 1L << logN1f;
        const int C = 1 << COLC;
        const int width = clampw(wmax);
        const int tiles = (width + C - 1) / C;
        ColFwdLegsCgArgs<T> a{};
        a.in = p1; a.FG = FG; a.FH = FH; a.lxd = lxd; a.lyd = lyd; a.gx = gx; a.gy = gy; a.h = h;
        a.pitch = pi; a.fpitch = kp; a.opitch = po; a.width = width; a.tw = tw_y; a.logTw = logNy; a.twc = cv.tw_y; a.n1f = N1f;
        a.in_moff = in_moff; a.out_moff = out_moff;
        q.col_fwdlegs_cg(tiles, (int)N1f, (int)((L * C) / EPT), ((size_t)L * C + tw_lds_size(logL) + 16 * C) * sizeof(cx<T>), logL, a,
                         nmaps > 1 ? 2 : 1);
        cx<T>* outs[3] = {gx, gy, h};
        const cx<T>* ins[3] = {gx, gy, h};
        cv.cols(q, gx, po, gx, po, width, true, (T)1, 2, 3, ins, outs, 0, false, 4, nmaps, out_moff, out_moff);
        return true;
    }

    static int div_lt() {
        static const int narrow = [] { const char* e = exp_env("OA_DIV_NARROW"); return e ? atoi(e) : 0; }();
        return (sizeof(T) == 4 ? 14 : 13) - (narrow > 0 ? 1 : 0);
    }
    static bool single_pass_div() {
        static const bool on = [] { const char* e = exp_env("OA_SINGLE_PASS_DIV"); return e ? atoi(e) != 0 : true; }();
        return on;
    }
    template <class Launcher>
    void cols_div(Launcher& q, const cx<T>* pa, const cx<T>* pb, const T* Fn, const T* lxd, const T* lyd, cx<T>* out,
                  cx<T>* tmpA, cx<T>* tmpB, int accumulate, int wmax = 0x7fffffff, int rband = 0, long pin = 0, int nmaps = 1,
                  long in_moff = 0, long tmp_moff = 0, long out_moff = 0, long fn_moff = 0) const {
        const long pi = pin > 0 ? pin : kp;
        if (single_pass_div() && (logNy == 10 || logNy == 11 || logNy == 12)) {
            const int lt = div_lt();
            const int lc = lt - logNy, Cs = 1 << lc;
            ColDivArgs<T> a{};
            a.A = pa; a.B = pb; a.Fn = Fn; a.lxd = lxd; a.lyd = lyd; a.out = out; a.pitch = pi; a.opitch = kp; a.width = clampw(wmax);
            a.logC = lc; a.NT = (1 << lt) / EPT; a.tw = tw_y; a.logTw = logNy; a.in_gs = 1; a.in_ns = 1; a.out_gs = 1; a.out_ks = 1;
            a.accumulate = accumulate; a.rband = clampr(rband); a.ny = ny; a.yshift = yshift();
            a.in_moff = in_moff; a.out_moff = out_moff; a.fn_moff = fn_moff;
            const int tl = (a.width + Cs - 1) / Cs;
            if (q.col_div_sp(tl, ((size_t)(1 << lt) + tw_lds_size(logNy)) * sizeof(cx<T>), logNy, a, nmaps)) return;
        }
        const int logN1 = (logNy + 1) / 2, logN2 = logNy - logN1;
        const long N1 = 1L << logN1, N2 = 1L << logN2;
        const int C = 1 << COLC;
        const int width = clampw(wmax);
        const int tiles = (width + C - 1) / C;
        const cx<T>* ins[2] = {pa, pb};
        cx<T>* outs[2] = {tmpA, tmpB};
        cols(q, pa, pi, tmpA, pi, width, false, (T)1, 1, 2, ins, outs, 0, false, -1, nmaps, in_moff, tmp_moff);
        ColDivArgs<T> a{};
        a.A = tmpA; a.B = tmpB; a.Fn = Fn; a.lxd = lxd; a.lyd = lyd; a.out = out; a.pitch = pi; a.opitch = kp; a.width = width;
        a.logC = COLC; a.NT = (int)((N2 * C) / EPT); if (a.NT < 1) a.NT = 1;
        a.tw = tw_y; a.logTw = logNy; a.in_gs = 1; a.in_ns = N1; a.out_gs = 1; a.out_ks = N1; a.accumulate = accumulate;
        a.rband = clampr(rband); a.ny = ny; a.yshift = yshift();
        a.in_moff = tmp_moff; a.out_moff = out_moff; a.fn_moff = fn_moff;
        q.col_div(tiles, (int)N1, a.NT, ((size_t)N2 * C + tw_lds_size(logN2) + N2) * sizeof(cx<T>), logN2, a, nmaps);
    }

    static int div3_logc(int rows) { return (sizeof(T) == 4 ? 3 : 2) + (rows == 768 ? 1 : 0); }
    template <class Launcher>
    void cols_div3(Launcher& q, const cx<T>* pa, const cx<T>* pb, const T* Fn, const T* lxd, const T* lyd, cx<T>* out, int accumulate,
                   int wmax = 0x7fffffff, int rband = 0, long pin = 0, int nmaps = 1, long in_moff = 0, long out_moff = 0, long fn_moff = 0) const {
        const int lc = div3_logc(ny), Cs = 1 << lc, logQ = ilog2(ny / 6);
        ColDivArgs<T> a{};
        a.A = pa; a.B = pb; a.Fn = Fn; a.lxd = lxd; a.lyd = lyd; a.out = out; a.pitch = pin > 0 ? pin : kp; a.opitch = kp; a.width = clampw(wmax);
        a.logC = lc; a.NT = 6 * (((ny / 6) << lc) / EPT); a.tw = tw_y; a.logTw = 0; a.in_gs = 1; a.in_ns = 1; a.out_gs = 1; a.out_ks = 1;
        a.accumulate = accumulate; a.rband = clampr(rband); a.ny = ny; a.yshift = yshift();
        a.in_moff = in_moff; a.out_moff = out_moff; a.fn_moff = fn_moff;
        q.col_div3((a.width + Cs - 1) / Cs, ((size_t)(ny << lc) + tw_lds_size(logQ)) * sizeof(cx<T>), ny, a, nmaps);
    }

    template <class Launcher>
    void r2c(Launcher& q, const T* in, cx<T>* out, cx<T>* tmp, T scale, int wmax = 0x7fffffff, int rband = 0) const {
        const int w = clampw(wmax);
        rows(q, ROW_R2C, in, nx / 2, tmp, kp, (T)1, w);
        cols(q, tmp, kp, out, kp, w, false, scale, 0, 1, nullptr, nullptr, rband);
    }
    template <class Launcher>
    void c2r(Launcher& q, const cx<T>* in, T* out, cx<T>* tmp, T scale, int wmax = 0x7fffffff, const T* mul = nullptr) const {
        const int w = clampw(wmax);
        cols(q, in, kp, tmp, kp, w, true, (T)1);
        rows(q, ROW_C2R, tmp, kp, out, nx / 2, scale, w, mul);
    }
    template <class Launcher>
    void c2c(Launcher& q, const cx<T>* in, cx<T>* out, cx<T>* tmp, bool inverse, T scale) const {
        rows(q, inverse ? ROW_C2C_I : ROW_C2C_F, in, nx, tmp, nx, (T)1);
        cols(q, tmp, nx, out, nx, nx, inverse, scale);
    }
};

}
```

### orphics_amd/csrc/pipeline.hip

```cpp
#include <dlfcn.h>
#include <cstdlib>
#include <algorithm>
#include <functional>
#include <string>
#include <utility>
#include <vector>
#include "common.hpp"
#include "fft_plan.hpp"

namespace oa {

constexpr int MC_BATCH_MAX = 6;

struct Pipeline {
    const void* FG = nullptr; const void* FH = nullptr; const void* Fn = nullptr;
    int wl = 0, wk = 0, rl = 0, rk = 0, mrow = -1;
    int mcol = -1;
    int my = 0;
    int my3 = 0;
    int map_grid() const { return my3 ? my3 : my; }
    void* work = nullptr;
    void* c[3] = {nullptr, nullptr, nullptr};
    void* g[2] = {nullptr, nullptr};
    void* kT = nullptr;
    void* kk = nullptr;
    const int32_t* ids = nullptr;
    int nids = 0;
    double norm = 1.0;
    void* bin_scratch = nullptr;
    double* sums = nullptr;
    int64_t* counts_full = nullptr;
    int64_t* counts_tmp = nullptr;
    unsigned* ticket = nullptr;
    void* split_legs = nullptr;
    size_t split_bytes = 0;
    void* mv_rtab = nullptr;
    std::vector<unsigned long long> mv_rkey;
    void* mc_src = nullptr;
    int mc_cap = 0;
    void* lens_pool = nullptr;
    size_t lens_bytes = 0;
    void* mvmc = nullptr;
    size_t mvmc_bytes = 0;
    void* mvwin = nullptr;
    size_t mvwin_bytes = 0;
    struct DivTabs {
        void* fn_t = nullptr; int32_t* ids_t = nullptr;
        size_t fn_t_bytes = 0, ids_t_bytes = 0;
        unsigned long tab_gen = 0;
        int tab_rows = 0, tab_logc = 0, tab_wk = 0;
    } dt[2];
    DivTabs& tabs_of(int rows) { return (my3 && rows == my3) ? dt[1] : dt[0]; }
    const DivTabs& tabs_of(int rows) const { return (my3 && rows == my3) ? dt[1] : dt[0]; }
    unsigned long bind_gen = 1;
    void* fb_t = nullptr;
    size_t fb_t_bytes = 0;
    unsigned long fb_gen = 0;
    int fb_my = 0, fb_wl = 0, fb_rl = 0;
    void** mv_ftab = nullptr;
    std::vector<const void*> mv_fkey;
    int opt_mc_batch = MC_BATCH_MAX;
    bool opt_mv_batch = true;
    bool opt_mv_rowbatch = true;
    bool opt_mv_chain = true;
    bool opt_divbin = true;
    bool opt_win_fused = true;
    bool opt_win_fused_set = false;
    oa_plan* band = nullptr;
    int bmy = 0, bmx = 0;
    void* bplanes = nullptr;
    int32_t* bids = nullptr;
    void* brows = nullptr;
    size_t brows_bytes = 0;
    void* bwin = nullptr;
    size_t bwin_bytes = 0;
    void* bsplit = nullptr;
    size_t bsplit_bytes = 0;
    int bs_cap = 0;
    void** bs_tab = nullptr;
    int bs_tab_cap = 0;
    std::vector<const void*> bs_key;
    struct PolBind {
        bool bound = false;
        oa_plan* plan = nullptr;
        int my = 0, mx = 0;
        int wl = 0, wk = 0, rl = 0, rk = 0, mrow = -1;
        std::vector<const void*> fkey, nkey;
        void* planes = nullptr;
        size_t planes_bytes = 0;
        void** stab = nullptr;
        std::vector<const void*> skey;
        void* mrows = nullptr;
        size_t mrows_bytes = 0;
        struct McBind {
            bool bound = false;
            const void* w = nullptr; long wstride = 0;
            const int32_t* ids = nullptr;
            int nids = 0, nest = 0, nspec_max = 0;
            void* pool = nullptr;
            size_t pool_bytes = 0, off_ids = 0, off_draw = 0, off_kappa = 0, off_scratch = 0, off_sums = 0;
        } mc;
    } pb;
};
constexpr int POL_SRC_MAX = 6;

static size_t plane_bytes(const oa_plan* p) { return (size_t)p->ny * p->kp * 2 * (p->dtype == OA_F32 ? 4 : 8); }

static Pipeline* pipe_of(oa_plan* p) {
    if (!p->pipe) p->pipe = new Pipeline();
    return (Pipeline*)p->pipe;
}

void pipeline_release(oa_plan* p) {
    if (!p || !p->pipe) return;
    Pipeline* q = (Pipeline*)p->pipe;
    if (q->work) (void)hipFree(q->work);
    if (q->bin_scratch) (void)hipFree(q->bin_scratch);
    if (q->sums) (void)hipFree(q->sums);
    if (q->counts_full) (void)hipFree(q->counts_full);
    if (q->counts_tmp) (void)hipFree(q->counts_tmp);
    if (q->ticket) (void)hipFree(q->ticket);
    if (q->split_legs) (void)hipFree(q->split_legs);
    if (q->mv_ftab) (void)hipFree(q->mv_ftab);
    if (q->mc_src) (void)hipFree(q->mc_src);
    if (q->mv_rtab) (void)hipFree(q->mv_rtab);
    if (q->lens_pool) (void)hipFree(q->lens_pool);
    if (q->mvmc) (void)hipFree(q->mvmc);
    if (q->mvwin) (void)hipFree(q->mvwin);
    for (auto& t : q->dt) { if (t.fn_t) (void)hipFree(t.fn_t); if (t.ids_t) (void)hipFree(t.ids_t); }
    if (q->fb_t) (void)hipFree(q->fb_t);
    if (q->band) (void)oa_plan_destroy(q->band);
    if (q->bplanes) (void)hipFree(q->bplanes);
    if (q->bids) (void)hipFree(q->bids);
    if (q->brows) (void)hipFree(q->brows);
    if (q->bwin) (void)hipFree(q->bwin);
    if (q->bsplit) (void)hipFree(q->bsplit);
    if (q->bs_tab) (void)hipFree(q->bs_tab);
    if (q->pb.plan) (void)oa_plan_destroy(q->pb.plan);
    if (q->pb.planes) (void)hipFree(q->pb.planes);
    if (q->pb.stab) (void)hipFree(q->pb.stab);
    if (q->pb.mrows) (void)hipFree(q->pb.mrows);
    if (q->pb.mc.pool) (void)hipFree(q->pb.mc.pool);
    delete q;
    p->pipe = nullptr;
}

static int ensure_work(oa_plan* p, Pipeline* q) {
    if (q->work) return 0;
// ... 66 lines not shown
    if (ok) {
        if (int rc = plan_ensure_col_grid(p, my3)) return rc;
        ok = qe_rsplit_lr(p, my3, q->wl, q->wk, q->mrow) == 2;
    }
    if (ok) q->my3 = my3;
    else if (want3) return fail("oa_plan_set_col_grid: this geometry has no from-map path on a 3 x 2^k column grid (built for 8192-row maps on 1536 "
                                "rows and 4096-row maps on 768 rows, R-split from-map path)");
    return 0;
}

}

using namespace oa;

static int ensure_div_tables(oa_plan* p, oa::Pipeline* q, hipStream_t st);
static int ensure_div_tables(oa_plan* p, oa::Pipeline* q, hipStream_t st, int rows);
namespace oa {
static int band_grid_rule(const oa_plan* p, int mrow, int mcol, int wl, int wk, int rl, int rk, int* my, int* mx);
static int mixed_bind(oa_plan* p, Pipeline* q);
static int mixed_bins(oa_plan* p, Pipeline* q, hipStream_t st);
static int mixed_qe_tt(oa_plan* p, Pipeline* q, const void* map, const void* kX, const void* kY, void* out, int zero_outside, hipStream_t st);
static int mixed_moments(oa_plan* p, Pipeline* q, const void* map, int64_t* n, double* S, double* C, hipStream_t st);
static int mixed_mc_run(oa_plan* p, Pipeline* q, uint64_t base_seed, long sim_lo, long sim_hi, const void* covsqrt_hc, int64_t* n, double* S,
                        double* C, double* meanfield_acc, hipStream_t st);
static int mixed_mc_run_windowed(oa_plan* p, Pipeline* q, uint64_t base_seed, long sim_lo, long sim_hi, const void* covsqrt_hc, const void* window,
                                 int64_t* n, double* S, double* C, double* meanfield_acc, hipStream_t st);
static void band_options(Pipeline* q);
struct MvCall {
    int nest; const int* npieces; const double* signs; const void* const* FG; const void* const* FH; const int* swap;
    const void* const* kX; const void* const* kY; const void* const* Fn; bool pol;
    int nmaps; const void* const* maps; const void* rot_c; const void* rot_s; const int* xsrc; const int* ysrc;
};
static int mixed_qe_mv(oa_plan* p, Pipeline* q, const MvCall& c, void* out, int accumulate, int wl, int wk, int rl, int rk, int mrow, int zero_outside,
                       hipStream_t st);
static int mixed_qe_tt_splits(oa_plan* p, Pipeline* q, const char* who, int nsplits, const void* const* host_kmaps, void* const* host_out,
                              void* out_power, double norm, int zero_outside, hipStream_t st);
}
#define OA_NOT_MIXED(p, what) \
    OA_REQUIRE(!(p)->mixed, what ": not available on map sides that are not powers of two (one-call TT entries there: oa_qe_tt, oa_qe_tt_moments(2), oa_mc_run)")

extern "C" {

int oa_plan_set_col_grid(oa_plan* p, int mcol) {
    OA_REQUIRE(p, "oa_plan_set_col_grid: NULL plan");
    OA_REQUIRE(p->pow2 || p->mixed, "oa_plan_set_col_grid: map sides with a prime factor other than 2, 3 and 5 (chirp-z transforms) have no one-call path");
    OA_REQUIRE(mcol <= 0 || is_pow2(mcol) || (is_m3(mcol) && p->pow2),
               "oa_plan_set_col_grid: mcol must be -1 (auto), 0 (off), a power of two, or 3 x 2^k (from-map path of power-of-two plans)");
    Pipeline* q = pipe_of(p);
    q->mcol = mcol;
    if (p->mixed) {
        if (!q->FG) return 0;
        int my = 0, mx = 0;
        int rc = band_grid_rule(p, q->mrow, q->mcol, q->wl, q->wk, q->rl, q->rk, &my, &mx);
        if (!rc && q->band && my == q->bmy && mx == q->bmx) return 0;
        if (!rc) rc = mixed_bind(p, q);
        if (rc) q->FG = nullptr;
        return rc;
    }
    return q->FG ? resolve_col_grid(p, q) : 0;
}

int oa_plan_col_grid(const oa_plan* p) { return (p && p->pipe) ? ((Pipeline*)p->pipe)->map_grid() : 0; }

int oa_plan_band_grid(const oa_plan* p, int* my, int* mx) {
    OA_REQUIRE(p && my && mx, "oa_plan_band_grid: NULL argument");
    const Pipeline* q = (const Pipeline*)p->pipe;
    const bool bound = q && q->FG && q->band;
    *my = bound ? q->bmy : 0;
    *mx = bound ? q->bmx : 0;
    return 0;
}

int oa_plan_set_option(oa_plan* p, int option, int value) {
    OA_REQUIRE(p, "oa_plan_set_option: NULL plan");
    Pipeline* q = pipe_of(p);
    switch (option) {
        case OA_OPT_MC_BATCH:
            OA_REQUIRE(value >= 0 && value <= MC_BATCH_MAX, "oa_plan_set_option: OA_OPT_MC_BATCH takes 0 (default) .. 6");
            q->opt_mc_batch = value ? value : MC_BATCH_MAX; return 0;
        case OA_OPT_MV_BATCH: q->opt_mv_batch = value != 0; return 0;
        case OA_OPT_MV_ROWBATCH: q->opt_mv_rowbatch = value != 0; return 0;
        case OA_OPT_MV_CHAIN: q->opt_mv_chain = value != 0; return 0;
        case OA_OPT_DIV_BIN: q->opt_divbin = value != 0; return 0;
        case OA_OPT_WIN_FUSED:
            q->opt_win_fused = value != 0; q->opt_win_fused_set = value >= 0; return 0;
        default: return fail("oa_plan_set_option: unknown option");
    }
}
}
namespace oa {
static void band_options(Pipeline* q) {
    for (oa_plan* inner : {q->band, q->pb.plan}) {
        if (!inner || !inner->pipe) continue;
        Pipeline* b = (Pipeline*)inner->pipe;
        b->opt_mc_batch = q->opt_mc_batch; b->opt_mv_batch = q->opt_mv_batch; b->opt_mv_rowbatch = q->opt_mv_rowbatch;
        b->opt_mv_chain = q->opt_mv_chain; b->opt_divbin = q->opt_divbin; b->opt_win_fused = q->opt_win_fused;
    }
}
}
extern "C" {
int oa_plan_rsplit(const oa_plan* p) {
    if (!p || !p->pipe) return 0;
    const Pipeline* q = (const Pipeline*)p->pipe;
    return q->FG ? (1 << qe_rsplit_lr(p, q->map_grid(), q->wl, q->wk, q->mrow)) & ~1 : 0;
}

int oa_plan_div_fused(const oa_plan* p) {
    if (!p || !p->pipe) return 0;
    const Pipeline* q = (const Pipeline*)p->pipe;
    if (p->mixed) { band_options((Pipeline*)q); return (q->FG && q->ids && q->band) ? oa_plan_div_fused(q->band) : 0; }
    if (!q->FG || !q->ids || !q->opt_divbin) return 0;
    const int rows = q->map_grid() ? q->map_grid() : p->ny;
    const bool sp = p->dtype == OA_F32 ? Fft2dPlan<float>::single_pass_div() : Fft2dPlan<double>::single_pass_div();
    if (!(sp && (rows == 1024 || rows == 2048 || rows == 4096 || (q->my3 && rows == q->my3)))) return 0;
    const int logc = div_tile_logc(p, rows);
    const long tiles = ((long)(q->wk > 0 ? q->wk : p->nx / 2 + 1) + (1 << logc) - 1) >> logc;
    return (tiles * MC_BATCH_MAX * q->nids <= (long)(oa_bin_scratch_bytes(q->nids) / 8) * MC_BATCH_MAX) ? 1 : 0;
}

int oa_plan_set_filters(oa_plan* p, const void* FG, const void* FH, const void* Fnorm, int leg_cols, int kappa_cols,
                        int leg_rows, int kappa_rows, int mrow) {
    OA_REQUIRE(p && FG && FH && Fnorm, "oa_plan_set_filters: NULL argument");
    OA_REQUIRE(p->pow2 || p->mixed, "oa_plan_set_filters: map sides with a prime factor other than 2, 3 and 5 (chirp-z transforms) have no "
               "one-call path (use the modular oa_qe_legs / oa_mul_real / oa_qe_div calls)");
    OA_REQUIRE(p->have_laxes, "oa_plan_set_filters: call oa_plan_set_laxes first");
    if (p->pow2) {
        const int hw = p->nx / 2 + 1;
        OA_REQUIRE(leg_cols <= hw && kappa_cols <= hw, "oa_plan_set_filters: leg / kappa columns beyond the hc plane (> nx / 2 + 1)");
        OA_REQUIRE(2L * leg_rows - 1 <= p->ny && 2L * kappa_rows - 1 <= p->ny, "oa_plan_set_filters: leg / kappa rows beyond the plane (2 rows - 1 > ny)");
    }
    Pipeline* q = pipe_of(p);
    q->FG = FG; q->FH = FH; q->Fn = Fnorm;
    ++q->bind_gen;
    q->wl = leg_cols; q->wk = kappa_cols; q->rl = leg_rows; q->rk = kappa_rows; q->mrow = mrow;
    q->mcol = mrow == 0 ? 0 : -1;
    if (int rc = ensure_work(p, q)) { if (p->mixed) q->FG = nullptr; return rc; }
    if (p->mixed) {
        int rc = mixed_bind(p, q);
        if (rc) q->FG = nullptr;
        return rc;
    }
    return resolve_col_grid(p, q);
}

int oa_plan_set_bins(oa_plan* p, const int32_t* ids_hc, int nids, double norm, void* stream) {
    OA_REQUIRE(p && ids_hc && nids >= 3, "oa_plan_set_bins: bad argument");
    Pipeline* q = pipe_of(p);
    if (int rc = ensure_work(p, q)) return rc;
    if (q->nids != nids) {
        if (q->bin_scratch) { OA_HIP(hipDeviceSynchronize()); (void)hipFree(q->bin_scratch); (void)hipFree(q->sums); (void)hipFree(q->counts_full); (void)hipFree(q->counts_tmp); }
        const long sb = oa_bin_scratch_bytes(nids);
        OA_REQUIRE(sb > 0, "oa_plan_set_bins: bad nids");
        OA_HIP(hipMalloc(&q->bin_scratch, (size_t)sb * MC_BATCH_MAX));
        OA_HIP(hipMalloc((void**)&q->sums, MC_BATCH_MAX * nids * sizeof(double)));
        OA_HIP(hipMalloc((void**)&q->counts_full, nids * sizeof(int64_t)));
        OA_HIP(hipMalloc((void**)&q->counts_tmp, MC_BATCH_MAX * nids * sizeof(int64_t)));
    }
    if (!q->ticket) {
        OA_HIP(hipMalloc((void**)&q->ticket, sizeof(unsigned)));
        OA_HIP(hipMemset(q->ticket, 0, sizeof(unsigned)));
    }
    q->ids = ids_hc; q->nids = nids; q->norm = norm;
    ++q->bind_gen;
    if (p->kp % 4 == 0) {
        if (int rc = oa_bin_power(p->dtype, q->c[0], q->c[0], norm, ids_hc, nullptr, (long)p->ny * p->kp, nids, p->kp, p->nx / 2, q->sums,
                                  q->counts_full, nullptr, q->bin_scratch, 0, 0, stream)) return rc;
    } else {
        const long kp4 = (p->kp + 3) / 4 * 4;
        const size_t es = 2 * (p->dtype == OA_F32 ? 4 : 8);
        int32_t* ids4 = nullptr;
        void* z4 = nullptr;
        OA_HIP(hipMalloc((void**)&ids4, (size_t)p->ny * kp4 * sizeof(int32_t)));
        hipError_t e = hipMalloc(&z4, (size_t)p->ny * kp4 * es);
        if (e == hipSuccess) e = hipMemsetAsync(ids4, 0xFF, (size_t)p->ny * kp4 * sizeof(int32_t), (hipStream_t)stream);
        if (e == hipSuccess) e = hipMemsetAsync(z4, 0, (size_t)p->ny * kp4 * es, (hipStream_t)stream);
        if (e == hipSuccess)
            e = hipMemcpy2DAsync(ids4, kp4 * sizeof(int32_t), ids_hc, p->kp * sizeof(int32_t), p->kp * sizeof(int32_t), p->ny, hipMemcpyDeviceToDevice,
                                 (hipStream_t)stream);
        int rc = e == hipSuccess ? oa_bin_power(p->dtype, z4, z4, norm, ids4, nullptr, (long)p->ny * kp4, nids, kp4, p->nx / 2, q->sums, q->counts_full,
// ... 440 lines not shown
                               host_signs[at] * s * s * sy, i > 0, leg_cols, kappa_cols, mrow, pl, pk, st, my);
            if (rc) return rc;
        }
        if (!dbatch)
            if (int rc = qe_cols_div_w(p, g0, g1, host_Fnorm[e], out, (accumulate || e > 0) ? 1 : 0, kappa_cols, kappa_rows, pk, st, my)) return rc;
    }
    if (dbatch) {
        if (int rc = qe_cols_div_batch_w(p, prod, prod + lbk, host_Fnorm[0], q->c[0], tmp, nest, (long)(2 * lbk / es), fn_moff, (long)(pb / es),
                                         kappa_cols, kappa_rows, pk, st, my)) return rc;
        if (keep_planes) return 0;
        const int wsum = (kappa_cols > 0 && kappa_cols <= p->nx / 2 + 1) ? kappa_cols : p->nx / 2 + 1;
        return sum_region(p->dtype, q->c[0], (long)(pb / es), nest, out, accumulate ? 1 : 0, p->ny, p->kp, wsum, kappa_rows, st);
    }
    return 0;
}

int oa_qe_tt_splits(oa_plan* p, int nsplits, const void* const* host_kmaps, void* const* host_out, int zero_outside, void* stream) {
    OA_REQUIRE(p && p->pipe && ((Pipeline*)p->pipe)->FG, "oa_qe_tt_splits: call oa_plan_set_filters first");
    OA_REQUIRE(nsplits >= 1 && nsplits <= 64 && host_kmaps && host_out, "oa_qe_tt_splits: bad argument");
    Pipeline* q = (Pipeline*)p->pipe;
    hipStream_t st = (hipStream_t)stream;
    if (p->mixed) return mixed_qe_tt_splits(p, q, "oa_qe_tt_splits", nsplits, host_kmaps, host_out, nullptr, 0.0, zero_outside, st);
    const long pl = work_pitch(p, q->wl), pk = work_pitch(p, q->wk);
    const size_t lb = (size_t)pl * p->ny * 2 * (p->dtype == OA_F32 ? 4 : 8);
    const size_t es = 2 * (p->dtype == OA_F32 ? 4 : 8), lbk = (size_t)pk * p->ny * es;
    const int npairs = nsplits * nsplits;
    bool dbatch = npairs >= 2 && q->opt_mv_batch;
    long out_moff = 0;
    if (dbatch) {
        const long d = (long)((char*)host_out[1] - (char*)host_out[0]);
        dbatch = d > 0 && d % (long)es == 0;
        for (int k = 2; k < npairs && dbatch; ++k) dbatch = host_out[k] && ((char*)host_out[k] - (char*)host_out[0]) == k * d;
        out_moff = d / (long)es;
    }
    if (int rc = ensure_pool(q, 3 * lb * nsplits + (dbatch ? 4 * (size_t)npairs * lbk : 0))) return rc;
    char* const prod = (char*)q->split_legs + 3 * lb * nsplits;
    const int my = q->my;
    auto leg = [&](int i, int c) { return (void*)((char*)q->split_legs + (3 * (size_t)i + c) * lb); };
    for (int i = 0; i < nsplits; ++i) {
        OA_REQUIRE(host_kmaps[i], "oa_qe_tt_splits: NULL split plane");
        if (int rc = qe_legs_cols_w(p, host_kmaps[i], host_kmaps[i], q->FG, q->FH, leg(i, 0), leg(i, 1), leg(i, 2), q->wl, q->rl, pl, st, my)) return rc;
    }
    const double s = 1.0 / ((double)p->ny * p->nx), sy = my ? (double)p->ny / my : 1.0;
    for (int i = 0; i < nsplits; ++i)
        for (int j = 0; j < nsplits; ++j) {
            const int k = i * nsplits + j;
            void* out = host_out[k];
            OA_REQUIRE(out, "oa_qe_tt_splits: NULL output plane");
            int rc;
            if (zero_outside && (rc = zero_complement(p, out, q->wk, q->rk, st))) return rc;
            void* g0 = dbatch ? (void*)(prod + 2 * (size_t)k * lbk) : q->g[0];
            void* g1 = dbatch ? (void*)(prod + (2 * (size_t)k + 1) * lbk) : q->g[1];
            if ((rc = qe_rows_w(p, leg(i, 0), leg(i, 1), leg(j, 2), g0, g1, s * s * sy, 0, q->wl, q->wk, q->mrow, pl, pk, st, my))) return rc;
            if (!dbatch && (rc = qe_cols_div_w(p, g0, g1, q->Fn, out, 0, q->wk, q->rk, pk, st, my))) return rc;
        }
    if (dbatch)
        return qe_cols_div_batch_w(p, prod, prod + lbk, q->Fn, host_out[0], prod + 2 * (size_t)npairs * lbk, npairs, (long)(2 * lbk / es), 0,
                                   out_moff, q->wk, q->rk, pk, st, my);
    return 0;
}

int oa_qe_tt_split_power(oa_plan* p, int nsplits, const void* const* host_kmaps, void* out_hcreal, double norm, int zero_outside, void* stream) {
    OA_REQUIRE(p && host_kmaps && out_hcreal, "oa_qe_tt_split_power: bad argument");
    OA_REQUIRE(nsplits >= 4 && nsplits <= 8, "oa_qe_tt_split_power: 4 <= nsplits <= 8");
    OA_REQUIRE(!p->pow2, "oa_qe_tt_split_power: a power-of-two plan has no band grid; there the estimate is oa_qe_tt_splits + oa_split_cross_power");
    OA_REQUIRE(p->pipe && ((Pipeline*)p->pipe)->FG, "oa_qe_tt_split_power: call oa_plan_set_filters first");
    return mixed_qe_tt_splits(p, (Pipeline*)p->pipe, "oa_qe_tt_split_power", nsplits, host_kmaps, nullptr, out_hcreal, norm, zero_outside,
                              (hipStream_t)stream);
}

int oa_qe_tt_moments2(oa_plan* p, const void* real_map0, const void* real_map1, int64_t* n, double* S, double* C, void* stream) {
    OA_REQUIRE(p && p->pipe && ((Pipeline*)p->pipe)->FG && ((Pipeline*)p->pipe)->ids, "oa_qe_tt_moments2: call oa_plan_set_filters and oa_plan_set_bins first");
    OA_REQUIRE(real_map0 && real_map1 && n && S && C, "oa_qe_tt_moments2: NULL argument");
    Pipeline* q = (Pipeline*)p->pipe;
    if (p->mixed) {
        if (int rc = mixed_moments(p, q, real_map0, n, S, C, (hipStream_t)stream)) return rc;
        return mixed_moments(p, q, real_map1, n, S, C, (hipStream_t)stream);
    }
    const long pl = work_pitch(p, q->wl), pk = work_pitch(p, q->wk);
    if (int rc = ensure_div_tables(p, q, (hipStream_t)stream)) return rc;
    DivBinFuse f = make_fuse(p, q, n, S, C, 0, q->map_grid());
    int rc = qe_tt_pair_w(p, real_map0, real_map1, q->FG, q->FH, q->Fn, q->c[0], q->c[1], q->c[2], q->g[0], q->g[1], q->kk, q->kT, q->wl,
                          q->wk, q->rl, q->rk, q->mrow, q->map_grid(), pl, pk, (hipStream_t)stream, divbin_enabled(q) ? &f : nullptr,
                          fband_table(p, q, (hipStream_t)stream));
    if (rc > 0) return rc;
    if (rc == 0 && f.done) return 0;
    if (rc < 0) {
        if ((rc = oa_qe_tt_moments(p, real_map0, n, S, C, stream))) return rc;
        return oa_qe_tt_moments(p, real_map1, n, S, C, stream);
    }
    const long es = 2 * (p->dtype == OA_F32 ? 4 : 8);
    const long back = ((const char*)q->kT - (const char*)q->kk) / es;
    return bin_power_moments(p->dtype, q->kk, q->norm, q->ids, (long)p->ny * p->kp, q->nids, p->kp, p->nx / 2, q->sums, q->counts_tmp,
                             q->bin_scratch, q->wk, q->rk, q->ticket, q->counts_full, n, S, C, (hipStream_t)stream, 2, back);
}

int oa_qe_tt_stage(oa_plan* p, int stage, const void* real_map, void* stream) {
    OA_REQUIRE(p && p->pipe && ((Pipeline*)p->pipe)->FG, "oa_qe_tt_stage: call oa_plan_set_filters first");
    OA_NOT_MIXED(p, "oa_qe_tt_stage");
    Pipeline* q = (Pipeline*)p->pipe;
    const long pl = work_pitch(p, q->wl), pk = work_pitch(p, q->wk);
    hipStream_t st = (hipStream_t)stream;
    const int my = q->map_grid();
    const double s = 1.0 / ((double)p->ny * p->nx), sy = my ? (double)p->ny / my : 1.0;
    const int lr = qe_rsplit_lr(p, my, q->wl, q->wk, q->mrow);
    switch (stage) {
        case 0: case 1: case 2:
            OA_REQUIRE(real_map, "oa_qe_tt_stage: stages 0-2 need the map");
            return qe_map_legs_cols_w(p, real_map, q->FG, q->FH, q->c[0], q->c[1], q->c[2], q->wl, q->rl, pl, st, 1 << stage, my, lr,
                                      lr ? fband_table(p, q, st) : nullptr);
        case 3: return qe_rows_w(p, q->c[0], q->c[1], q->c[2], q->g[0], q->g[1], s * s * sy, 0, q->wl, q->wk, q->mrow, pl, pk, st, my, lr);
        case 4: {
            if (q->ids && divbin_enabled(q)) {
                DivBinFuse f = make_fuse(p, q, (int64_t*)q->kT, (double*)q->kT + 8, (double*)q->kT + 8 + q->nids, 0, my);
                return qe_cols_div_w(p, q->g[0], q->g[1], q->Fn, q->kk, 0, q->wk, q->rk, pk, st, my, &f);
            }
            return qe_cols_div_w(p, q->g[0], q->g[1], q->Fn, q->kk, 0, q->wk, q->rk, pk, st, my);
        }
        case 5: {
            OA_REQUIRE(q->ids, "oa_qe_tt_stage: stage 5 needs oa_plan_set_bins");
            if (oa_plan_div_fused(p)) return 0;
            int64_t* n = (int64_t*)q->kT;
            double* S = (double*)q->kT + 8;
            double* C = S + q->nids;
            return bandpower_moments(p, q, n, S, C, stream);
        }
        default: return fail("oa_qe_tt_stage: stage must be 0..5");
    }
}

}

namespace oa {
static int ensure_mc_src(oa_plan* p, Pipeline* q) {
    if (q->mc_cap >= MC_BATCH_MAX) return 0;
    if (q->mc_src) { OA_HIP(hipDeviceSynchronize()); (void)hipFree(q->mc_src); q->mc_src = nullptr; q->mc_cap = 0; }
    OA_HIP(hipMalloc(&q->mc_src, (size_t)MC_BATCH_MAX * plane_bytes(p)));
    q->mc_cap = MC_BATCH_MAX;
    return 0;
}
static size_t mc_pool_bytes(const oa_plan* p, const Pipeline* q, int B) {
    const size_t es = 2 * (p->dtype == OA_F32 ? 4 : 8);
    return 3 * (size_t)B * work_pitch(p, q->wl) * p->ny * es + 4 * (size_t)B * work_pitch(p, q->wk) * p->ny * es;
}
static int mc_batch_tail(oa_plan* p, Pipeline* q, int B, int64_t* n, double* S, double* C, double* meanfield_acc, hipStream_t st, int* fallback,
                         bool keep_kappa = false) {
    *fallback = 0;
    const long pl = work_pitch(p, q->wl), pk = work_pitch(p, q->wk);
    const size_t es = 2 * (p->dtype == OA_F32 ? 4 : 8), pb = plane_bytes(p);
    const size_t lb = (size_t)pl * p->ny * es, lbk = (size_t)pk * p->ny * es;
    const int my = q->my;
    if (int rc = ensure_pool(q, mc_pool_bytes(p, q, B))) return rc;
    char* const legs = (char*)q->split_legs;
    char* const prod = legs + 3 * (size_t)B * lb;
    char* const tmp = prod + 2 * (size_t)B * lbk;
    std::vector<const void*> key;
    for (int b = 0; b < B; ++b) key.push_back(q->FG);
    for (int b = 0; b < B; ++b) key.push_back(q->FH);
    if (!q->mv_ftab) OA_HIP(hipMalloc((void**)&q->mv_ftab, 32 * sizeof(void*)));
    if (key != q->mv_fkey) {
        OA_HIP(hipMemcpyAsync(q->mv_ftab, key.data(), key.size() * sizeof(void*), hipMemcpyHostToDevice, st));
        q->mv_fkey = key;
    }
    unsigned long long sel = 0;
    for (int f = 0; f < 2 * B; ++f) sel |= (unsigned long long)(f % B) << (4 * f);
    const double s = 1.0 / ((double)p->ny * p->nx), sy = my ? (double)p->ny / my : 1.0;
    int legs_done = 0, rc;
// ... 895 lines not shown
```

### orphics_amd/engine.py

```python
import ctypes

import numpy as np
import torch

from . import _lib
from ._lib import OA_F32, OA_F64, check


def _ptr(t):
    return ctypes.c_void_p(t.data_ptr()) if t is not None else None


def _stream():
    return ctypes.c_void_p(torch.cuda.current_stream().cuda_stream)


def _dirty(t):
    mark_dirty(t)
    return t


_RDT = {"f32": torch.float32, "f64": torch.float64}
_CDT = {"f32": torch.complex64, "f64": torch.complex128}
_CODE = {"f32": OA_F32, "f64": OA_F64}
# ... 304 lines not shown

    def fft_pass(self, pass_id, src, dst, width=0):
        check(self.lib.oa_fft_pass(self.plan, int(pass_id), _ptr(src), _ptr(dst), int(width), _stream()))

    def hc_to_full(self, k):
        self._chk(k, "hc")
        out = self.full()
        check(self.lib.oa_hc_to_full(self.plan, _ptr(k), _ptr(out), _stream()))
        return out

    def full_to_hc(self, z):
        self._chk(z, "full")
        out = self.hc()
        check(self.lib.oa_full_to_hc(self.plan, _ptr(z), _ptr(out), _stream()))
        return out

    def hcreal_to_full(self, f):
        self._chk(f, "hcreal")
        out = self.real()
        check(self.lib.oa_hcreal_to_full(self.plan, _ptr(f), _ptr(out), _stream()))
        return out

    def fullreal_to_hc(self, f):
        self._chk(f, "real")
        out = self.hcreal()
        check(self.lib.oa_fullreal_to_hc(self.plan, _ptr(f), _ptr(out), _stream()))
        return out

    def _same(self, *ts):
        n = ts[0].numel()
        for t in ts:
            if not (isinstance(t, torch.Tensor) and t.is_cuda and t.is_contiguous() and t.numel() == n):
                raise ValueError("elementwise operands must be contiguous CUDA tensors of equal size")
        return n

    def f2power(self, k1, k2, norm, out=None):
        n = self._same(k1, k2)
        if k1.dtype != self.cdt or k2.dtype != self.cdt:
            raise ValueError("f2power: complex dtype mismatch")
        out = torch.empty(k1.shape, dtype=self.rdt, device=self.device) if out is None else _dirty(out)
        check(self.lib.oa_f2power(self.code, _ptr(k1), _ptr(k2), _ptr(out), float(norm), n, _stream()))
        return out

    def cmul_real(self, k, f, out=None):
        n = self._same(k, f)
        if k.dtype != self.cdt or f.dtype != self.rdt:
            raise ValueError("cmul_real: dtype mismatch")
        out = torch.empty_like(k) if out is None else _dirty(out)
        check(self.lib.oa_cmul_real(self.code, _ptr(k), _ptr(f), _ptr(out), n, _stream()))
        return out

    def cmul(self, k, f, out=None):
        n = self._same(k, f)
        if k.dtype != self.cdt or f.dtype != self.cdt:
            raise ValueError("cmul: dtype mismatch")
        out = torch.empty_like(k) if out is None else _dirty(out)
        check(self.lib.oa_cmul(self.code, _ptr(k), _ptr(f), _ptr(out), n, _stream()))
        return out

    def mul_real(self, a, b, out=None):
        n = self._same(a, b)
        if a.dtype != self.rdt or b.dtype != self.rdt:
            raise ValueError("mul_real: dtype mismatch")
        out = torch.empty_like(a) if out is None else _dirty(out)
        check(self.lib.oa_mul_real(self.code, _ptr(a), _ptr(b), _ptr(out), n, _stream()))
        return out

    def axpby(self, a, b, alpha, beta, out=None):
        n = self._same(a, b)
        if a.dtype != self.rdt or b.dtype != self.rdt:
            raise ValueError("axpby: dtype mismatch")
        out = torch.empty_like(a) if out is None else _dirty(out)
        check(self.lib.oa_axpby_real(self.code, _ptr(a), _ptr(b), _ptr(out), float(alpha), float(beta), n, _stream()))
        return out

    def rot2(self, c, s, i1, i2):
        n = self._same(c, s, i1, i2)
        if c.dtype != self.rdt or i1.dtype != self.cdt or i2.dtype != self.cdt or s.dtype != self.rdt:
            raise ValueError("rot2: dtype mismatch")
        o1, o2 = torch.empty_like(i1), torch.empty_like(i2)
        check(self.lib.oa_rot2(self.code, _ptr(c), _ptr(s), _ptr(i1), _ptr(i2), _ptr(o1), _ptr(o2), n, _stream()))
        return o1, o2

    OPTIONS = {"mc_batch": 1, "mv_batch": 2, "mv_rowbatch": 3, "mv_chain": 4, "div_bin": 5, "win_fused": 6}

    def set_option(self, name, value):
        if name not in self.OPTIONS:
            raise ValueError("unknown plan option %r (one of %s)" % (name, sorted(self.OPTIONS)))
        check(self.lib.oa_plan_set_option(self.plan, self.OPTIONS[name], int(value)))
        self._options = dict(getattr(self, "_options", {}), **{name: int(value)})

    def copy_options_to(self, other):
        for name, value in getattr(self, "_options", {}).items():
            other.set_option(name, value)

    def band_grid(self, leg_cols, kappa_cols, leg_rows, kappa_rows, mrow=-1, mcol=-1):
        if not self.mixed:
            return None
        return band_grid(self.ny, self.nx, leg_cols, kappa_cols, leg_rows, kappa_rows, mrow, mcol)

    def plan_band_grid(self):
        my, mx = ctypes.c_int(0), ctypes.c_int(0)
        check(self.lib.oa_plan_band_grid(self.plan, ctypes.byref(my), ctypes.byref(mx)))
        return my.value, mx.value

    def release_pools(self):
        check(self.lib.oa_plan_release_pools(self.plan))
        self._mc_owner = None

    def set_laxes(self, ly, lx):
        ly = np.ascontiguousarray(ly, dtype=np.float64)
        lx = np.ascontiguousarray(lx, dtype=np.float64)
        if ly.shape != (self.ny,) or lx.shape != (self.nx,):
            raise ValueError("laxes must have shapes (ny,), (nx,)")
        check(self.lib.oa_plan_set_laxes(self.plan, ly.ctypes.data_as(ctypes.c_void_p), lx.ctypes.data_as(ctypes.c_void_p)))
        self._laxes = (ly, lx)

    def qe_legs(self, kX, kY, FG, FH, phase_g=0, phase_h=0, h_times_i=False, out=None):
        self._chk(kX, "hc"); self._chk(kY, "hc"); self._chk(FG, "hcreal"); self._chk(FH, "hcreal")
        if out is None:
            out = (self.hc(), self.hc(), self.hc())
        Gx, Gy, H = out
        _dirty(Gx); _dirty(Gy); _dirty(H)
        check(self.lib.oa_qe_legs(self.plan, _ptr(kX), _ptr(kY), _ptr(FG), _ptr(FH), _ptr(Gx), _ptr(Gy), _ptr(H),
                                  int(phase_g), int(phase_h), 1 if h_times_i else 0, _stream()))
        return Gx, Gy, H

    def qe_div(self, Px, Py, Fnorm, out=None, accumulate=False):
        self._chk(Px, "hc"); self._chk(Py, "hc"); self._chk(Fnorm, "hcreal")
        out = self.hc() if out is None else _dirty(self._chk(out, "hc"))
        check(self.lib.oa_qe_div(self.plan, _ptr(Px), _ptr(Py), _ptr(Fnorm), _ptr(out), 1 if accumulate else 0, _stream()))
        return out

    def lens_split(self, alpha, step):
        self._chk(alpha, "real")
        shift = torch.empty(alpha.shape, dtype=torch.int32, device=self.device)
        delta = torch.empty_like(alpha)
        check(self.lib.oa_lens_split(self.code, _ptr(alpha), float(step), _ptr(shift), _ptr(delta), alpha.numel(), _stream()))
        return shift, delta

    def lens_gather(self, src, sx, sy, dx, dy, px, py, coef, out, accumulate):
        self._chk(src, "real"); _dirty(self._chk(out, "real")); self._chk(dx, "real"); self._chk(dy, "real")
        if sx.dtype != torch.int32 or sy.dtype != torch.int32 or sx.numel() != src.numel() or sy.numel() != src.numel():
            raise ValueError("lens_gather: shifts must be int32 planes")
        check(self.lib.oa_lens_gather(self.plan, _ptr(src), _ptr(sx), _ptr(sy), _ptr(dx), _ptr(dy), int(px), int(py),
                                      float(coef), _ptr(out), 1 if accumulate else 0, _stream()))
        return out

    def digitize(self, x64, edges64):
        return dev_digitize(x64, edges64)

    def modl_digitize(self, edges64, half=False, want_modl=False):
        if self._laxes is None:
            raise RuntimeError("set_laxes first")
        ly = torch.as_tensor(self._laxes[0], device=self.device)
        lx = torch.as_tensor(self._laxes[1], device=self.device)
        pitch, width = (self.kp, self.nxh + 1) if half else (self.nx, self.nx)
        ids = torch.empty((self.ny, pitch), dtype=torch.int32, device=self.device)
        modl = torch.empty((self.ny, pitch), dtype=torch.float64, device=self.device) if want_modl else None
        check(self.lib.oa_modl_digitize(_ptr(ly), _ptr(lx), self.ny, self.nx, pitch, width, _ptr(edges64),
                                        edges64.numel(), _ptr(ids), _ptr(modl), _stream()))
        return (ids, modl) if want_modl else ids

    def bin(self, data, ids, nids, weights=None, aux=None, mode=0, skip_nan=False, herm=False):
        return dev_bin(data, ids, nids, weights=weights, aux=aux, mode=mode, skip_nan=skip_nan,
                       herm_pitch=self.kp if herm else 0, herm_nxh=self.nxh if herm else -1)

# ... 121 lines not shown
```

Baseline: 5843.

## Process both maps of a TT pair per workgroup in the fused divergence-binning kernel

Adds a mode where one workgroup of the 3x2^k column divergence kernel handles several maps (two by default for f64 pairs), looping over them. The next map's global loads are issued before the current map's bin accumulation, so load latency can overlap the atomic binning. Per-map per-wave bin rows live in extra LDS and are folded in a single finish. This cuts the workgroup count and finish/ticket overhead, at the cost of more LDS per workgroup (capped at 160 KiB, with fallback) and higher register pressure, which may lower occupancy.

```diff
diff --git a/include/orphics_amd.h b/include/orphics_amd.h
--- a/include/orphics_amd.h
+++ b/include/orphics_amd.h
@@ -14,7 +14,7 @@
 typedef struct oa_plan oa_plan;
 
 const char* oa_last_error(void);
-#define OA_ABI_VERSION 409
+#define OA_ABI_VERSION 410
 int oa_version(void);
 int oa_device_count(void);
 
@@ -51,7 +51,8 @@
 int oa_qe_band_grid(const oa_plan* p, int* my, int* mx);
 int oa_plan_rsplit(const oa_plan* p);
 int oa_plan_div_fused(const oa_plan* p);
-enum { OA_OPT_MC_BATCH = 1, OA_OPT_MV_BATCH = 2, OA_OPT_MV_ROWBATCH = 3, OA_OPT_MV_CHAIN = 4, OA_OPT_DIV_BIN = 5, OA_OPT_WIN_FUSED = 6 };
+enum { OA_OPT_MC_BATCH = 1, OA_OPT_MV_BATCH = 2, OA_OPT_MV_ROWBATCH = 3, OA_OPT_MV_CHAIN = 4, OA_OPT_DIV_BIN = 5, OA_OPT_WIN_FUSED = 6,
+       OA_OPT_DIV_MAPS = 7 };
 int oa_plan_set_option(oa_plan* p, int option, int value);
 int oa_plan_set_bins(oa_plan* p, const int32_t* ids_hc, int nids, double norm, void* stream);
 void* oa_plan_kappa(oa_plan* p);
diff --git a/orphics_amd/_lib.py b/orphics_amd/_lib.py
--- a/orphics_amd/_lib.py
+++ b/orphics_amd/_lib.py
@@ -6,7 +6,7 @@
 
 OA_F32 = 0
 OA_F64 = 1
-ABI_VERSION = 409
+ABI_VERSION = 410
 
 c_void_p = ctypes.c_void_p
 c_int = ctypes.c_int
diff --git a/orphics_amd/csrc/common.hpp b/orphics_amd/csrc/common.hpp
--- a/orphics_amd/csrc/common.hpp
+++ b/orphics_amd/csrc/common.hpp
@@ -48,6 +48,7 @@
     const int64_t* mcounts; int64_t* n; double* S; double* C;
     int store;
     int gx;
+    int nmaps;
     bool done;
 };
 
@@ -160,7 +161,7 @@
                   long pk, hipStream_t st, int my = 0, DivBinFuse* fuse = nullptr);
 int qe_tt_pair_w(oa_plan* p, const void* map0, const void* map1, const void* FG, const void* FH, const void* Fn, void* c0, void* c1,
                  void* c2, void* g0, void* g1, void* out0, void* out1, int wl, int wk, int rl, int rk, int mrow, int my, long pl, long pk,
-                 hipStream_t st, DivBinFuse* fuse = nullptr, const void* fgh = nullptr);
+                 hipStream_t st, DivBinFuse* fuse = nullptr, const void* fgh = nullptr, int div_maps = 0);
 int band_map_r2c(oa_plan* p, const void* map, void* rowbuf, int wl, int rl, void* dst, int dny, long dkp, hipStream_t st);
 size_t band_map_scratch_bytes(const oa_plan* p, int wl, int rl);
 int band_maps_r2c(oa_plan* p, int nmaps, const void* const* maps, const void* rot_c, const void* rot_s, void* scratch, int wl, int rl, void* dst,
diff --git a/orphics_amd/csrc/fft.hip b/orphics_amd/csrc/fft.hip
--- a/orphics_amd/csrc/fft.hip
+++ b/orphics_amd/csrc/fft.hip
@@ -469,6 +469,7 @@
             if (e != hipSuccess) { rc = fail(std::string("hipFuncSetAttribute: ") + hipGetErrorString(e)); return; }
         }
         fuse->gx = gx;
+        fuse->nmaps = a.wg_maps > 0 ? a.nmaps : gz;
         if (!fuse->store) a.out = nullptr;
         const bool tabs = fuse->tab_logc == a.logC && fuse->tab_rows == a.ny;
         a.Fn_t = (tabs && a.fn_moff == 0) ? (const T*)fuse->fn_t : nullptr;
@@ -501,12 +502,18 @@
         return false;
     }
     template <typename T>
-    void col_div3(int gx, size_t smem, int rows, const ColDivArgs<T>& a, int gz = 1) {
+    void col_div3(int gx, size_t smem, int rows, const ColDivArgs<T>& a_in, int gz = 1) {
         if (rc) return;
         constexpr int lc = sizeof(T) == 4 ? 3 : 2;
         if (rows != 1536 && rows != 768) { rc = fail("fft: unsupported 3 x 2^k divergence grid"); return; }
-        const int nt = a.NT;
-        if (fuse && !a.accumulate && (long)gx * gz * fuse->nids <= fuse->part_cap &&
+        ColDivArgs<T> a = a_in;
+        const int nt = a.NT, nmaps = a.wg_maps > 0 ? a.nmaps : gz;
+        if (fuse && a.wg_maps > 0) {
+            const size_t need = smem + (size_t)a.wg_maps * (nt / 64) * fuse->nids * sizeof(double);
+            if (need <= (size_t)160 * 1024) smem = need;
+            else { a.wg_maps = 0; a.nmaps = 0; gz = nmaps; }
+        }
+        if (fuse && !a.accumulate && (long)gx * nmaps * fuse->nids <= fuse->part_cap &&
             (size_t)(nt / 64) * fuse->nids * sizeof(double) <= ((size_t)rows << a.logC) * sizeof(cx<T>)) {
             if (rows == 1536) go_fused(col_div3_sp_bin_kernel<T, 8, lc>, gx, gz, nt, smem, a);
             else go_fused(col_div3_sp_bin_kernel<T, 7, lc + 1>, gx, gz, nt, smem, a);
@@ -761,10 +768,17 @@
     return q.rc;
 }
 
+static int div_maps_per_wg(int elem_bytes, int rows, int tiles, int nmaps, int forced) {
+    (void)rows; (void)tiles;
+    if (nmaps < 2) return 1;
+    if (forced > 0) return forced < nmaps ? forced : nmaps;
+    return (elem_bytes == 8 && nmaps == 2) ? 2 : 1;
+}
+
 template <typename T>
 static int qe_tt_pair_impl(oa_plan* p, const void* map0, const void* map1, const void* FG, const void* FH, const void* Fn, void* c0,
                            void* c1, void* c2, void* g0, void* g1, void* out0, void* out1, int wl, int wk, int rl, int rk, int mrow,
-                           int my, long pl, long pk, hipStream_t st, DivBinFuse* fuse, const void* fgh) {
+                           int my, long pl, long pk, hipStream_t st, DivBinFuse* fuse, const void* fgh, int div_maps) {
     auto f = view<T>(p);
     const int lr = rsplit_lr<T>(p, my, wl, wk, mrow);
     const bool m3 = is_m3(my);
@@ -796,8 +810,11 @@
                      pl, 2, ms, cms, (const cx<T>*)fgh);
         cv.rows_qe(q, (const cx<T>*)c0, (const cx<T>*)c1, (const cx<T>*)c2, (cx<T>*)g0, (cx<T>*)g1, (T)(s * s * sy), 0, wi, wo, mrow, pl, pk, 2, cms, gms,
                    -1, nullptr, lr);
-        if (m3) cv.cols_div3(q, (const cx<T>*)g0, (const cx<T>*)g1, (const T*)Fn, (const T*)p->lxd, (const T*)p->lyd, (cx<T>*)out0, 0, wk, rk, pk, 2, gms,
-                             (long)((cx<T>*)out1 - (cx<T>*)out0));
+        if (m3) {
+            const int Cs = 1 << Fft2dPlan<T>::div3_logc(my);
+            cv.cols_div3(q, (const cx<T>*)g0, (const cx<T>*)g1, (const T*)Fn, (const T*)p->lxd, (const T*)p->lyd, (cx<T>*)out0, 0, wk, rk, pk, 2, gms,
+                         (long)((cx<T>*)out1 - (cx<T>*)out0), 0, div_maps_per_wg((int)sizeof(T), my, (wo + Cs - 1) / Cs, 2, div_maps));
+        }
         else
         cv.cols_div(q, (const cx<T>*)g0, (const cx<T>*)g1, (const T*)Fn, (const T*)p->lxd, (const T*)p->lyd, (cx<T>*)out0, tA, tB, 0, wk, rk, pk, 2,
                     gms, gms, (long)((cx<T>*)out1 - (cx<T>*)out0));
@@ -818,9 +835,9 @@
 }
 int qe_tt_pair_w(oa_plan* p, const void* map0, const void* map1, const void* FG, const void* FH, const void* Fn, void* c0, void* c1,
                  void* c2, void* g0, void* g1, void* out0, void* out1, int wl, int wk, int rl, int rk, int mrow, int my, long pl, long pk,
-                 hipStream_t st, DivBinFuse* fuse, const void* fgh) {
-    return p->dtype == OA_F32 ? qe_tt_pair_impl<float>(p, map0, map1, FG, FH, Fn, c0, c1, c2, g0, g1, out0, out1, wl, wk, rl, rk, mrow, my, pl, pk, st, fuse, fgh)
-                              : qe_tt_pair_impl<double>(p, map0, map1, FG, FH, Fn, c0, c1, c2, g0, g1, out0, out1, wl, wk, rl, rk, mrow, my, pl, pk, st, fuse, fgh);
+                 hipStream_t st, DivBinFuse* fuse, const void* fgh, int div_maps) {
+    return p->dtype == OA_F32 ? qe_tt_pair_impl<float>(p, map0, map1, FG, FH, Fn, c0, c1, c2, g0, g1, out0, out1, wl, wk, rl, rk, mrow, my, pl, pk, st, fuse, fgh, div_maps)
+                              : qe_tt_pair_impl<double>(p, map0, map1, FG, FH, Fn, c0, c1, c2, g0, g1, out0, out1, wl, wk, rl, rk, mrow, my, pl, pk, st, fuse, fgh, div_maps);
 }
 template <typename T>
 static int fband_pack_impl(oa_plan* p, const void* FG, const void* FH, void* out, int width, int rband, int my, hipStream_t st) {
diff --git a/orphics_amd/csrc/fft_divbin.hpp b/orphics_amd/csrc/fft_divbin.hpp
--- a/orphics_amd/csrc/fft_divbin.hpp
+++ b/orphics_amd/csrc/fft_divbin.hpp
@@ -33,21 +33,24 @@
     static constexpr bool active = true;
     DivBinFuse f;
     double* rows = nullptr;
+    double* fold = nullptr;
 
-    __device__ __forceinline__ void begin(GpuCtx&, void* lds) {
-        rows = reinterpret_cast<double*>(lds);
+    __device__ __forceinline__ void begin(GpuCtx& c, void* lds) { begin(c, lds, lds, 1); }
+    __device__ __forceinline__ void begin(GpuCtx&, void* tile, void* rws, int slots) {
+        fold = reinterpret_cast<double*>(tile);
+        rows = reinterpret_cast<double*>(rws);
         const int nw = blockDim.x >> 6;
-        for (int i = threadIdx.x; i < nw * f.nids; i += blockDim.x) rows[i] = 0.0;
+        for (int i = threadIdx.x; i < slots * nw * f.nids; i += blockDim.x) rows[i] = 0.0;
     }
     __device__ __forceinline__ int id_at(unsigned yfull, int col) const { return f.ids[(long)yfull * f.ipitch + col]; }
     __device__ __forceinline__ bool packed_ids() const { return f.ids_t != nullptr; }
     __device__ __forceinline__ int id_at_t(long i) const { return f.ids_t[i]; }
-    __device__ __forceinline__ void add(GpuCtx&, int id, T pw, int col) {
+    __device__ __forceinline__ void add(GpuCtx&, int id, T pw, int col, int row0 = 0) {
         const int m = (col == 0 || col == f.nxh) ? 1 : (col < f.nxh ? 2 : 0);
         const bool ok = id >= 0 && id < f.nids && m > 0;
         const double v = ok ? (double)(pw * (T)f.pnorm) * (double)m : 0.0;
         const int lane = threadIdx.x & 63;
-        double* row = rows + (threadIdx.x >> 6) * f.nids;
+        double* row = rows + (row0 + (int)(threadIdx.x >> 6)) * f.nids;
         unsigned long long act = __ballot(ok);
         while (act) {
             const int leader = __ffsll((long long)act) - 1;
@@ -59,15 +62,17 @@
             act &= ~mm;
         }
     }
-    __device__ __forceinline__ void finish(GpuCtx&) {
+    __device__ __forceinline__ void finish(GpuCtx& c) { finish(c, (int)blockIdx.z, 1); }
+    __device__ __forceinline__ void finish(GpuCtx&, int z0, int nz) {
         __shared__ int s_last;
         const int t = threadIdx.x, nt = blockDim.x, nw = nt >> 6, nids = f.nids;
         __syncthreads();
-        const long wg = (long)blockIdx.z * gridDim.x + blockIdx.x;
-        for (int i = t; i < nids; i += nt) {
+        for (int e = t; e < nz * nids; e += nt) {
+            const int m = e / nids, i = e - m * nids;
+            const double* rm = rows + m * nw * nids;
             double s = 0.0;
-            for (int k = 0; k < nw; ++k) s += rows[k * nids + i];
-            __hip_atomic_store(f.part + wg * nids + i, s, __ATOMIC_RELAXED, __HIP_MEMORY_SCOPE_AGENT);
+            for (int k = 0; k < nw; ++k) s += rm[k * nids + i];
+            __hip_atomic_store(f.part + ((long)(z0 + m) * gridDim.x + blockIdx.x) * nids + i, s, __ATOMIC_RELAXED, __HIP_MEMORY_SCOPE_AGENT);
         }
         asm volatile("s_waitcnt vmcnt(0)" ::: "memory");
         __syncthreads();
@@ -79,9 +84,9 @@
         int NI = 1;
         while (NI < nids && NI < nt) NI <<= 1;
         const int G = nt / NI > 0 ? nt / NI : 1, gi = t / NI, ii = t - gi * NI;
-        double* red = rows;
+        double* red = fold;
         const int gx = (int)gridDim.x;
-        for (int z = 0; z < (int)gridDim.z; ++z) {
+        for (int z = 0; z < f.nmaps; ++z) {
             for (int i0 = 0; i0 < nids; i0 += NI) {
                 const int i = i0 + ii;
                 __syncthreads();
@@ -121,7 +126,7 @@
             }
         }
         if (t == 0) {
-            if (f.n) f.n[0] += (int64_t)gridDim.z;
+            if (f.n) f.n[0] += (int64_t)f.nmaps;
             __hip_atomic_store(f.ticket, 0u, __ATOMIC_RELAXED, __HIP_MEMORY_SCOPE_AGENT);
         }
     }
diff --git a/orphics_amd/csrc/fft_kernels.hpp b/orphics_amd/csrc/fft_kernels.hpp
--- a/orphics_amd/csrc/fft_kernels.hpp
+++ b/orphics_amd/csrc/fft_kernels.hpp
@@ -1505,16 +1505,19 @@
     long in_moff, out_moff;
     long fn_moff;
     const T* Fn_t;
+    int wg_maps, nmaps;
 };
 
 struct NoDivTail {
     static constexpr bool active = false;
     template <class Ctx> OA_HD void begin(Ctx&, void*) {}
+    template <class Ctx> OA_HD void begin(Ctx&, void*, void*, int) {}
     OA_HD int id_at(unsigned, int) const { return -1; }
     OA_HD bool packed_ids() const { return false; }
     OA_HD int id_at_t(long) const { return -1; }
-    template <class Ctx, typename T> OA_HD void add(Ctx&, int, T, int) {}
+    template <class Ctx, typename T> OA_HD void add(Ctx&, int, T, int, int = 0) {}
     template <class Ctx> OA_HD void finish(Ctx&) {}
+    template <class Ctx> OA_HD void finish(Ctx&, int, int) {}
 };
 
 template <typename T, class SEQ, class Ctx, int LOGC = COL_LOGC, class Tail = NoDivTail>
@@ -1646,6 +1649,30 @@
     for (int q = 0; q < 3; ++q) { v[q] = e[q] + o[q]; v[q + 3] = e[q] - o[q]; }
 }
 
+template <typename T, int R>
+OA_HD void stage_in_loads(cx<T>* v, int tid, int NT, int logL, int logC, const ColLoad<T>& ld) {
+    constexpr int LR = Log2c<R>::v;
+    constexpr int NB = EPT / R;
+    const int logLR = logL - LR;
+#pragma unroll
+    for (int u = 0; u < NB; ++u) {
+        const int b = tid + u * NT;
+        const int c = b & ((1 << logC) - 1), j = b >> logC;
+        const int cc = c < ld.ncols ? c : ld.ncols - 1;
+#pragma unroll
+        for (int t = 0; t < R; ++t) {
+            const int n = j + (t << logLR);
+            const cx<T> x = ld.base[(unsigned)n * ld.nstride + (unsigned)cc];
+            v[u * R + t] = ld.inv ? swp(x) : x;
+        }
+    }
+}
+template <typename T, int R>
+OA_HD void stage_in_dfts(cx<T>* v) {
+#pragma unroll
+    for (int u = 0; u < EPT / R; ++u) Dft<T, R>::run(v + u * R);
+}
+
 template <typename T, int LOGQ, int LOGC, class Ctx, class Tail = NoDivTail>
 OA_HD void col_div3_body(Ctx& ctx, const ColDivArgs<T>& a, Tail tail = Tail{}) {
     cx<T>* s = reinterpret_cast<cx<T>*>(ctx.smem());
@@ -1666,28 +1693,40 @@
     if (ncols > C) ncols = C;
     cx<T>* twl = s + (N << logC);
     tw_lds_fill_mul<T>(ctx, twl, a.tw, 6, LOGQ, NT);
-    const long zmap = ctx.bid_z();
-    const long imo = zmap * a.in_moff, omo = zmap * a.out_moff;
-    const int grp = tid / NTS, tq = tid - grp * NTS;
+    const int wgm = a.wg_maps > 0 ? a.wg_maps : 1;
+    const int z0 = (int)ctx.bid_z() * wgm;
+    const int z1 = a.wg_maps > 0 ? (z0 + wgm < a.nmaps ? z0 + wgm : a.nmaps) : z0 + 1;
+    cx<T> va[EPT], vb[EPT];
+    auto loads = [&](int z, int t) {
+        const int grp = t / NTS, tq = t - grp * NTS;
+        const cx<T>* org = a.A + (long)z * a.in_moff + (long)grp * a.pitch + c0;
+        const ColLoad<T> la{org, (unsigned)(6 * a.pitch), ncols, false};
+        const ColLoad<T> lb{a.B + (org - a.A), (unsigned)(6 * a.pitch), ncols, false};
+        stage_in_loads<T, R0>(va, tq, NTS, LOGQ, logC, la);
+        stage_in_loads<T, R0>(vb, tq, NTS, LOGQ, logC, lb);
+    };
+    if constexpr (Tail::active) loads(z0, tid);
+    int tz = tid;
+    for (int z = z0; z < z1; ++z) {
+    if constexpr (!Tail::active) loads(z, tz);
+    stage_in_dfts<T, R0>(va);
+    stage_in_dfts<T, R0>(vb);
+    ctx.sync();
+    tz += (int)reinterpret_cast<const volatile T*>(twl)[1];
+    const int grp = tz / NTS, tq = tz - grp * NTS;
     cx<T>* sr = s + grp * (Q << logC);
-    const ColLoad<T> la{a.A + imo + (long)grp * a.pitch + c0, (unsigned)(6 * a.pitch), ncols, false};
-    const ColLoad<T> lb{a.B + imo + (long)grp * a.pitch + c0, (unsigned)(6 * a.pitch), ncols, false};
     int pk[NIT], pc[NIT];
     bool pv[NIT];
     cx<T> w1[NIT], w2[NIT], w4[NIT];
 #pragma unroll
     for (int it = 0; it < NIT; ++it) {
-        const int i = tid + it * NT;
+        const int i = tz + it * NT;
         pv[it] = i < (Q << logC);
-        const int ii = pv[it] ? i : tid;
+        const int ii = pv[it] ? i : tz;
         pc[it] = ii & (C - 1); pk[it] = ii >> logC;
         w1[it] = ldg(a.tw + pk[it]); w2[it] = ldg(a.tw + 2 * pk[it]); w4[it] = ldg(a.tw + 4 * pk[it]);
     }
-    cx<T> va[EPT], vb[EPT];
     cx<T> xa[NIT][6], xb[NIT][6];
-    stage_in<T, R0, false, true>(s, va, tq, NTS, LOGQ, logC, 0, 0, twl, LOGQ, la);
-    stage_in<T, R0, false, true>(s, vb, tq, NTS, LOGQ, logC, 0, 0, twl, LOGQ, lb);
-    ctx.sync();
     auto finish = [&](cx<T>* v, cx<T> (*x)[6]) {
         stage_out<T, R0, false, false>(sr, v, tq, NTS, LOGQ, logC, 0, 0, NoStore{});
         ctx.sync();
@@ -1706,12 +1745,14 @@
     finish(va, xa);
     ctx.sync();
     finish(vb, xb);
-    const T* Fnb = a.Fn + zmap * a.fn_moff + c0;
-    cx<T>* outb = a.out + omo + c0;
+    const T* Fnb = a.Fn + z * a.fn_moff + c0;
+    cx<T>* outb = a.out + z * a.out_moff + c0;
     if constexpr (Tail::active) {
-        ctx.sync();
-        tail.begin(ctx, s);
-        ctx.sync();
+        if (z == z0) {
+            ctx.sync();
+            tail.begin(ctx, s, a.wg_maps > 0 ? (void*)(twl + tw_lds_size(LOGQ)) : (void*)s, z1 - z0);
+            ctx.sync();
+        }
         T pw[NIT * 6];
         int idv[NIT * 6];
 #pragma unroll
@@ -1736,16 +1777,21 @@
                         outb[i] = d;
                     }
                     pw[it * 6 + q] = d.x * d.x + d.y * d.y;
-                    idv[it * 6 + q] = tail.packed_ids() ? tail.id_at_t(ti_) : tail.id_at(y + up, c0 + c);
+                    const int id = tail.packed_ids() ? tail.id_at_t(ti_) : tail.id_at(y + up, c0 + c);
+                    idv[it * 6 + q] = id < -1 ? -1 : id;
                 }
             }
         }
+        if (z + 1 < z1) loads(z + 1, tz);
+        else {
+#pragma unroll
+            for (int i = 0; i < EPT; ++i) va[i] = vb[i] = mk<T>((T)0, (T)0);
+        }
 #pragma unroll
         for (int it = 0; it < NIT; ++it) {
 #pragma unroll
-            for (int q = 0; q < 6; ++q) tail.add(ctx, idv[it * 6 + q], pw[it * 6 + q], c0 + pc[it]);
-        }
-        tail.finish(ctx);
+            for (int q = 0; q < 6; ++q) tail.add(ctx, idv[it * 6 + q], pw[it * 6 + q], c0 + pc[it], (z - z0) * (NT / 64));
+        }
     } else {
 #pragma unroll
         for (int it = 0; it < NIT; ++it) {
@@ -1764,6 +1810,8 @@
             }
         }
     }
+    }
+    if constexpr (Tail::active) tail.finish(ctx, z0, z1 - z0);
 }
 
 template <typename T>
diff --git a/orphics_amd/csrc/fft_plan.hpp b/orphics_amd/csrc/fft_plan.hpp
--- a/orphics_amd/csrc/fft_plan.hpp
+++ b/orphics_amd/csrc/fft_plan.hpp
@@ -432,14 +432,20 @@
     static int div3_logc(int rows) { return (sizeof(T) == 4 ? 3 : 2) + (rows == 768 ? 1 : 0); }
     template <class Launcher>
     void cols_div3(Launcher& q, const cx<T>* pa, const cx<T>* pb, const T* Fn, const T* lxd, const T* lyd, cx<T>* out, int accumulate,
-                   int wmax = 0x7fffffff, int rband = 0, long pin = 0, int nmaps = 1, long in_moff = 0, long out_moff = 0, long fn_moff = 0) const {
+                   int wmax = 0x7fffffff, int rband = 0, long pin = 0, int nmaps = 1, long in_moff = 0, long out_moff = 0, long fn_moff = 0,
+                   int div_maps = 0) const {
         const int lc = div3_logc(ny), Cs = 1 << lc, logQ = ilog2(ny / 6);
         ColDivArgs<T> a{};
         a.A = pa; a.B = pb; a.Fn = Fn; a.lxd = lxd; a.lyd = lyd; a.out = out; a.pitch = pin > 0 ? pin : kp; a.opitch = kp; a.width = clampw(wmax);
         a.logC = lc; a.NT = 6 * (((ny / 6) << lc) / EPT); a.tw = tw_y; a.logTw = 0; a.in_gs = 1; a.in_ns = 1; a.out_gs = 1; a.out_ks = 1;
         a.accumulate = accumulate; a.rband = clampr(rband); a.ny = ny; a.yshift = yshift();
         a.in_moff = in_moff; a.out_moff = out_moff; a.fn_moff = fn_moff;
-        q.col_div3((a.width + Cs - 1) / Cs, ((size_t)(ny << lc) + tw_lds_size(logQ)) * sizeof(cx<T>), ny, a, nmaps);
+        int gz = nmaps;
+        if (div_maps > 1 && nmaps > 1) {
+            a.wg_maps = div_maps < nmaps ? div_maps : nmaps; a.nmaps = nmaps;
+            gz = (nmaps + a.wg_maps - 1) / a.wg_maps;
+        }
+        q.col_div3((a.width + Cs - 1) / Cs, ((size_t)(ny << lc) + tw_lds_size(logQ)) * sizeof(cx<T>), ny, a, gz);
     }
 
     template <class Launcher>
diff --git a/orphics_amd/csrc/pipeline.hip b/orphics_amd/csrc/pipeline.hip
--- a/orphics_amd/csrc/pipeline.hip
+++ b/orphics_amd/csrc/pipeline.hip
@@ -64,6 +64,7 @@
     bool opt_mv_rowbatch = true;
     bool opt_mv_chain = true;
     bool opt_divbin = true;
+    int opt_div_maps = 0;
     bool opt_win_fused = true;
     bool opt_win_fused_set = false;
     oa_plan* band = nullptr;
@@ -296,6 +297,9 @@
         case OA_OPT_MV_ROWBATCH: q->opt_mv_rowbatch = value != 0; return 0;
         case OA_OPT_MV_CHAIN: q->opt_mv_chain = value != 0; return 0;
         case OA_OPT_DIV_BIN: q->opt_divbin = value != 0; return 0;
+        case OA_OPT_DIV_MAPS:
+            OA_REQUIRE(value >= 0 && value <= MC_BATCH_MAX, "oa_plan_set_option: OA_OPT_DIV_MAPS takes 0 (policy) .. 6");
+            q->opt_div_maps = value; return 0;
         case OA_OPT_WIN_FUSED:
             q->opt_win_fused = value != 0; q->opt_win_fused_set = value >= 0; return 0;
         default: return fail("oa_plan_set_option: unknown option");
@@ -309,6 +313,7 @@
         Pipeline* b = (Pipeline*)inner->pipe;
         b->opt_mc_batch = q->opt_mc_batch; b->opt_mv_batch = q->opt_mv_batch; b->opt_mv_rowbatch = q->opt_mv_rowbatch;
         b->opt_mv_chain = q->opt_mv_chain; b->opt_divbin = q->opt_divbin; b->opt_win_fused = q->opt_win_fused;
+        b->opt_div_maps = q->opt_div_maps;
     }
 }
 }
@@ -915,7 +920,7 @@
     DivBinFuse f = make_fuse(p, q, n, S, C, 0, q->map_grid());
     int rc = qe_tt_pair_w(p, real_map0, real_map1, q->FG, q->FH, q->Fn, q->c[0], q->c[1], q->c[2], q->g[0], q->g[1], q->kk, q->kT, q->wl,
                           q->wk, q->rl, q->rk, q->mrow, q->map_grid(), pl, pk, (hipStream_t)stream, divbin_enabled(q) ? &f : nullptr,
-                          fband_table(p, q, (hipStream_t)stream));
+                          fband_table(p, q, (hipStream_t)stream), q->opt_div_maps);
     if (rc > 0) return rc;
     if (rc == 0 && f.done) return 0;
     if (rc < 0) {
diff --git a/orphics_amd/engine.py b/orphics_amd/engine.py
--- a/orphics_amd/engine.py
+++ b/orphics_amd/engine.py
@@ -410,7 +410,7 @@
         check(self.lib.oa_rot2(self.code, _ptr(c), _ptr(s), _ptr(i1), _ptr(i2), _ptr(o1), _ptr(o2), n, _stream()))
         return o1, o2
 
-    OPTIONS = {"mc_batch": 1, "mv_batch": 2, "mv_rowbatch": 3, "mv_chain": 4, "div_bin": 5, "win_fused": 6}
+    OPTIONS = {"mc_batch": 1, "mv_batch": 2, "mv_rowbatch": 3, "mv_chain": 4, "div_bin": 5, "win_fused": 6, "div_maps": 7}
 
     def set_option(self, name, value):
         if name not in self.OPTIONS:
```

Result: no change. 5892 (median of 6 runs) (+0.8%).
